# sglang-npu/DeepGEMM_Ascend

Hardware: AMD Instinct MI355X
Metric: fp8 TFLOPS + % MFMA peak, 4096^3 block-scaled GEMM; grouped-GEMM tok/s at 1/2/4/8 GPU (higher is better)
Workload: dtype bf16

## Files before the change

deepgemm_ascend_amd/csrc/dga_launch.hip:

```cpp
#include <hip/hip_runtime.h>
#include <atomic>
#include <cstdio>
#include <cstdlib>
#include <cstring>
#include <mutex>

#include "dga_hip.h"
#include "dga_internal.hpp"
#include "dga_fp8_menu_impl.hpp"
#include "gemm_fp8_aux_kernels.hpp"

namespace dga {

static std::atomic<int> g_last_hip_error{0};
int record_hip(hipError_t e)
{
    if (e != hipSuccess) {
        g_last_hip_error.store(static_cast<int>(e));
        return DGA_E_HIP;
    }
    return DGA_OK;
}
uint32_t device_cus()
{
    static std::atomic<uint32_t> cache[64];
    int dev = 0, n = 0;
    if (hipGetDevice(&dev) != hipSuccess || dev < 0 || dev >= 64) return 256;
    if (const uint32_t v = cache[dev].load()) return v;
    if (hipDeviceGetAttribute(&n, hipDeviceAttributeMultiprocessorCount, dev) != hipSuccess || n <= 0) return 256;
    cache[dev].store(static_cast<uint32_t>(n));
    return static_cast<uint32_t>(n);
}

struct Variant {
    int bm, bn, wm, wn;
    int (*launch)(const GemmParams &, hipStream_t);
    int lds;
    int (*launch_pp)(const GemmParams &, hipStream_t);
    int (*launch_cont)(const GemmParams &, hipStream_t);
    int stages = 2;
    int (*launch_lc)(const GemmParams &, hipStream_t) = nullptr;
    int (*launch_ps)(const GemmParams &, hipStream_t) = nullptr;
};

#define DGA_VARIANT(BM, BN, WM, WN) \
    Variant { BM, BN, WM, WN, &launch_cfg<GemmCfg<BM, BN, WM, WN>, 0>, GemmCfg<BM, BN, WM, WN>::LDS_BYTES, nullptr, nullptr }
#define DGA_VARIANT_C(BM, BN, WM, WN) \
    Variant { BM, BN, WM, WN, &launch_cfg<GemmCfg<BM, BN, WM, WN>, 0>, GemmCfg<BM, BN, WM, WN>::LDS_BYTES, nullptr, \
              &launch_cfg<GemmCfg<BM, BN, WM, WN>, 2> }
#define DGA_VARIANT_PP(BM, BN, WM, WN)                                                                       \
    Variant { BM, BN, WM, WN, &launch_cfg<GemmCfg<BM, BN, WM, WN>, 0>, GemmCfg<BM, BN, WM, WN>::LDS_BYTES, \
              &launch_cfg<GemmCfg<BM, BN, WM, WN>, 1>, &launch_cfg<GemmCfg<BM, BN, WM, WN>, 2> }

static const Variant kVariants[] = {
    DGA_VARIANT_PP(256, 256, 4, 2), DGA_VARIANT_C(128, 256, 2, 2), DGA_VARIANT_C(256, 128, 4, 1),
    DGA_VARIANT_C(128, 128, 2, 2), DGA_VARIANT_C(64, 256, 1, 4),  DGA_VARIANT(64, 128, 1, 4),
    DGA_VARIANT_C(128, 256, 2, 4),
    Variant{128, 256, 2, 4, &launch_cfg<GemmCfg<128, 256, 2, 4, 3>, 0>, GemmCfg<128, 256, 2, 4, 3>::LDS_BYTES, nullptr, nullptr, 3},
    Variant{128, 256, 2, 2, &launch_cfg<GemmCfg<128, 256, 2, 2, 3>, 0>, GemmCfg<128, 256, 2, 2, 3>::LDS_BYTES, nullptr, nullptr, 3,
            &launch_cfg<GemmCfg<128, 256, 2, 2, 3, 4>, 0>, &launch_persistent<GemmCfg<128, 256, 2, 2, 3, 4>>},
    Variant{128, 128, 2, 2, &launch_cfg<GemmCfg<128, 128, 2, 2, 3>, 0>, GemmCfg<128, 128, 2, 2, 3>::LDS_BYTES, nullptr, nullptr, 3,
            &launch_cfg<GemmCfg<128, 128, 2, 2, 3, 4>, 0>, &launch_persistent<GemmCfg<128, 128, 2, 2, 3, 4>>},
    Variant{64, 256, 1, 4, &launch_cfg<GemmCfg<64, 256, 1, 4, 3>, 0>, GemmCfg<64, 256, 1, 4, 3>::LDS_BYTES, nullptr, nullptr, 3,
            &launch_cfg<GemmCfg<64, 256, 1, 4, 3, 4>, 0>, &launch_persistent<GemmCfg<64, 256, 1, 4, 3, 4>>},

    DGA_VARIANT(32, 256, 1, 4),  DGA_VARIANT(32, 128, 1, 4),  DGA_VARIANT(16, 256, 1, 4),
    DGA_VARIANT(16, 128, 1, 4),
    Variant{64, 128, 1, 4, &launch_cfg<GemmCfg<64, 128, 1, 4, 3>, 0>, GemmCfg<64, 128, 1, 4, 3>::LDS_BYTES, nullptr, nullptr, 3,
            &launch_cfg<GemmCfg<64, 128, 1, 4, 3, 4>, 0>, &launch_persistent<GemmCfg<64, 128, 1, 4, 3, 4>>},
    Variant{32, 256, 1, 4, &launch_cfg<GemmCfg<32, 256, 1, 4, 3>, 0>, GemmCfg<32, 256, 1, 4, 3>::LDS_BYTES, nullptr, nullptr, 3},
    Variant{32, 128, 1, 4, &launch_cfg<GemmCfg<32, 128, 1, 4, 3>, 0>, GemmCfg<32, 128, 1, 4, 3>::LDS_BYTES, nullptr, nullptr, 3},
    Variant{16, 256, 1, 4, &launch_cfg<GemmCfg<16, 256, 1, 4, 3>, 0>, GemmCfg<16, 256, 1, 4, 3>::LDS_BYTES, nullptr, nullptr, 3},
    Variant{16, 128, 1, 4, &launch_cfg<GemmCfg<16, 128, 1, 4, 3>, 0>, GemmCfg<16, 128, 1, 4, 3>::LDS_BYTES, nullptr, nullptr, 3,
            &launch_cfg<GemmCfg<16, 128, 1, 4, 3, 4>, 0>, &launch_persistent<GemmCfg<16, 128, 1, 4, 3, 4>>},
};
static constexpr int kNumVariants = sizeof(kVariants) / sizeof(kVariants[0]);

struct Bf16xVariant {
    int bm, bn;
    int (*launch[3])(const GemmParams &, hipStream_t);
    int (*launch_kgroup)(const GemmParams &, hipStream_t);
};
#define DGA_BX_VARIANT(BM, BN, WM, WN) {BM, BN, {&launch_bf16x<GemmCfg<BM, BN, WM, WN, 3>>, &launch_bf16x_f32<GemmCfg<BM, BN, WM, WN, 3>>, \
                                         &launch_bf16x_rows<GemmCfg<BM, BN, WM, WN, 3>>}, &launch_bf16x_kgroup<GemmCfg<BM, BN, WM, WN, 3>>}
static const Bf16xVariant kBf16xVariants[] = {
    DGA_BX_VARIANT(128, 256, 2, 4), DGA_BX_VARIANT(128, 128, 2, 2), DGA_BX_VARIANT(64, 256, 1, 4), DGA_BX_VARIANT(64, 128, 1, 4),
    DGA_BX_VARIANT(32, 128, 1, 4),
};
static const Bf16xVariant *find_bf16x_variant(int m1, int n1)
{
    const int bm = m1 >= 128 ? 128 : (m1 >= 64 ? 64 : 32);
    const int bn = n1 >= 256 ? 256 : 128;
    for (const auto &v : kBf16xVariants)
        if (v.bm == bm && v.bn == bn) return &v;
    for (const auto &v : kBf16xVariants)
        if (v.bm == bm) return &v;
    return nullptr;
}

static const char *const kPolicyNames[] = {"fast", "bf16_exact", "strict", "fast_ue8m0", "bf16_exact_ue8m0", "auto"};
int default_policy()
{
    static const int v = [] {
        const char *e = std::getenv("DGA_DEFAULT_POLICY");
        if (!e || !*e) return 1;
        for (int i = 0; i < 6; ++i)
            if (!std::strcmp(e, kPolicyNames[i])) return i;
        return -1;
    }();
    return v;
}

int variant_count() { return kNumVariants; }
int variant_stages(int i) { return kVariants[i].stages; }
bool variant_has_loader_waves(int i) { return kVariants[i].launch_lc != nullptr; }
void variant_info(int i, int *bm, int *bn, int *wm, int *wn, int *lds)
{
    *bm = kVariants[i].bm; *bn = kVariants[i].bn; *wm = kVariants[i].wm; *wn = kVariants[i].wn;
    *lds = kVariants[i].lds;
}

static const Variant *find_variant(int bm, int bn, int wm, int wn, int stages)
{
    for (int i = 0; i < kNumVariants; ++i)
        if (kVariants[i].bm == bm && kVariants[i].bn == bn && (!wm || (kVariants[i].wm == wm && kVariants[i].wn == wn)) &&
            kVariants[i].stages == (stages == 3 ? 3 : 2))
            return &kVariants[i];
    if (stages == 3) return find_variant(bm, bn, wm, wn, 2);
    return wm ? find_variant(bm, bn, 0, 0, 2) : nullptr;
}

static int check_tiling(const dga_tiling_t &t)
{
    if (t.dispatchPolicyTag & ~(DGA_POLICY_UE8M0_SCALES | 7)) return DGA_E_TILING;
    const int tag = t.dispatchPolicyTag & 7;
    if (!known_kernel_serial(t.kernelSerial)) return DGA_E_TILING;
    if (t.k1 != 0 && t.k1 != 128) return DGA_E_TILING;
    if (t.splitkFactor > 1024) return DGA_E_RANGE;
    if (t.reserved0) return DGA_E_TILING;
    if (tag == DGA_POLICY_STRICT) return DGA_OK;
    if (t.m1 == 0 || t.n1 == 0) return DGA_E_TILING;
    if (!(t.stages == 0 || t.stages == 2 || t.stages == 3)) return DGA_E_TILING;
    const bool wsk = t.kernelSerial == DGA_KERNEL_SPLITK_WORKGROUP;
    if (t.build == DGA_BUILD_WSK_REGISTER && !wsk) return DGA_E_TILING;
    if (tag == DGA_POLICY_BF16_EXACT) {
        if (!find_bf16x_variant(t.m1, t.n1)) return DGA_E_TILING;
        switch (t.build) {
            case DGA_BUILD_DEFAULT: case DGA_BUILD_WSK_REGISTER: case DGA_BUILD_BX_AIMAGE: case DGA_BUILD_BX_IMAGE8: case DGA_BUILD_BX_IMAGE4:
            case DGA_BUILD_BX_PERSISTENT: case DGA_BUILD_BX_ONE_TILE: case DGA_BUILD_BX_GROUPED: break;
            case DGA_BUILD_BX_DECODE:
                if (!wsk || t.m1 != 64 || t.n1 != 128) return DGA_E_TILING;
                break;
            default: return DGA_E_TILING;
        }
        if ((t.kernelSerial == DGA_KERNEL_STREAMK_TAIL || t.kernelSerial == DGA_KERNEL_STREAMK_ONE_LAUNCH) && !(t.m1 >= 128 && t.n1 >= 256)) return DGA_E_TILING;
        return DGA_OK;
    }
    bool tile = false, grid = false;
    for (int i = 0; i < kNumVariants; ++i)
        if (kVariants[i].bm == t.m1 && kVariants[i].bn == t.n1) {
            tile = true;
            if (kVariants[i].wm == t.wavesM && kVariants[i].wn == t.wavesN) grid = true;
        }
    if (!tile) return DGA_E_TILING;
    if (t.m1 == 256 && t.n1 == 256 && t.wavesM == 2 && t.wavesN == 2 && (t.dispatchPolicyTag & DGA_POLICY_UE8M0_SCALES) &&
        (tag == DGA_POLICY_CONTINUOUS || tag == DGA_POLICY_CONTINUOUS_PERSISTENT))
        grid = true;
    if ((t.wavesM || t.wavesN) && !grid) return DGA_E_TILING;
    if (t.build != DGA_BUILD_DEFAULT && t.build != DGA_BUILD_WSK_REGISTER) return DGA_E_TILING;
    if (tag == DGA_POLICY_PINGPONG && !(t.m1 == 256 && t.n1 == 256)) return DGA_E_TILING;
    if ((t.kernelSerial == DGA_KERNEL_STREAMK_TAIL || t.kernelSerial == DGA_KERNEL_STREAMK_ONE_LAUNCH) && !(t.m1 == 256 && t.n1 == 256))
        return DGA_E_TILING;
    return DGA_OK;
}

static int (*find_clock_build(const Variant *v, int policy))(const GemmParams &, hipStream_t)
{
    if (v->bm == 256 && v->bn == 256 && policy == DGA_POLICY_CONTINUOUS) return &launch_cfg<GemmCfg<256, 256, 4, 2, 2>, 2, true>;
    if (v->bm == 128 && v->bn == 256 && v->stages == 3 && policy == DGA_POLICY_LOADER_WAVES) return &launch_cfg<GemmCfg<128, 256, 2, 2, 3, 4>, 0, true>;
    return nullptr;
}

struct Switches {
    int bf16_exact = env_int("DGA_BF16_EXACT", 0);
    int strict = env_int("DGA_STRICT", 0);
    int b_nt = env_int("DGA_B_NT", -1), out_nt = env_int("DGA_OUT_NT", -1);
    int unaligned = env_int("DGA_UNALIGNED", -1);
    int xcd_remap = env_int("DGA_XCD_REMAP", 1);
    int bx_image = env_int("DGA_BX_IMAGE", -1);
    int wsk = env_int("DGA_WSK", -1), wsk_dma = env_int("DGA_WSK_DMA", -1);
    int pingpong = env_int("DGA_PINGPONG", -1);
    int bx_persist = env_int("DGA_BF16X_PERSIST", -1), bx_grouped = env_int("DGA_BX_GROUPED", -1);
};
static const Switches &env()
{
    static const Switches s;
    return s;
}

static int strict_bm(int groups, int m, int n)
{
    const int64_t tiles64 = static_cast<int64_t>(groups) * ((m + 63) / 64) * ((n + 127) / 128);
    return (m > 32 && tiles64 >= static_cast<int64_t>(device_cus())) ? 64 : 32;
}

static bool partial_overlap(const float *c, const float *out, uintptr_t bytes)
{
    if (!c || c == out) return false;
    const uintptr_t co = reinterpret_cast<uintptr_t>(c), oo = reinterpret_cast<uintptr_t>(out);
    return co < oo + bytes && oo < co + bytes;
}

static dga_problem_t fp8_problem(int m, int n, int k, int groups)
{
    dga_problem_t pr{};
    pr.m = m; pr.n = n; pr.k = k; pr.groups = groups;
    pr.layoutTagA = DGA_LAYOUT_ROW_MAJOR; pr.layoutTagB = DGA_LAYOUT_COLUMN_MAJOR;
    pr.layoutTagC = DGA_LAYOUT_ROW_MAJOR; pr.dtype = DGA_DT_FP8_E4M3FN;
    return pr;
}

static int check_tiling_for(Out kind, const dga_tiling_t *t)
{
    if (kind == Out::F32Rows) return dga_tiling_check_wgrad(t);
    if (kind == Out::F32) return dga_tiling_check_fp32_out(t);
    return check_tiling(*t);
}

struct Carver {
    uint8_t *ws;
    size_t bytes, used = 0;
    uint8_t *operator()(size_t n)
    {
        const size_t at = (used + 255) & ~size_t(255);
        if (!ws || at + n > bytes) return nullptr;
        used = at + n;
        return ws + at;
    }
};


static int resolve_tiling(const Fp8Call &c, dga_tiling_t &local)
{
    dga_problem_t pr = fp8_problem(c.m, c.n, c.k, c.groups);
    pr.expected_m = c.expected_m;
    pr.flags = c.m_indices ? DGA_PROBLEM_CONTIGUOUS_M : 0;
    if (c.kind == Out::F32) return dga_tiling_fp32_out(&pr, &local);
    if (c.kind == Out::F32Rows) return dga_tiling_wgrad(&pr, &local);
    const int default_policy = dga::default_policy();
    if (default_policy < 0) return DGA_E_RANGE;
    const int rc = (env().bf16_exact || default_policy == 1 || default_policy == 4) ? dga_tiling_bf16_exact(&pr, &local) : dga_tiling(&pr, &local);
    if (rc != DGA_OK) return rc;
    if (default_policy == 5 && c.groups == 1 && !c.m_indices) {
        dga_tiling_t tb;
        if (dga_tiling_bf16_exact(&pr, &tb) == DGA_OK && tb.kernelSerial == DGA_KERNEL_SPLITK_WORKGROUP) local = tb;
    }
    if (default_policy == 2) local.dispatchPolicyTag = DGA_POLICY_STRICT;
    if (default_policy == 3 || default_policy == 4) local.dispatchPolicyTag |= DGA_POLICY_UE8M0_SCALES;
    return DGA_OK;
}

static int fill_params(const Fp8Call &c, GemmParams &p)
{
    const int m = c.m, n = c.n, k = c.k;
    p.a = static_cast<const uint8_t *>(c.a);
    p.sfa = c.sfa;
    p.b = static_cast<const uint8_t *>(c.b);
    p.sfb = c.sfb;
    p.out = static_cast<uint16_t *>(c.out);
    p.masked_m = c.masked_m;
    p.m_indices = c.m_indices;
    p.b_groups = c.b_groups;
    p.m = m; p.n = n; p.k = k;
    p.kb_n = (k + 127) / 128;
    p.nb_n = c.kind == Out::F32Rows ? n : (n + 127) / 128;
    p.lda = k; p.ldb = k; p.ldc = n;
    p.a_gs = static_cast<int64_t>(m) * k;
    p.b_gs = static_cast<int64_t>(n) * k;
    p.c_gs = static_cast<int64_t>(m) * n;
    p.sfa_gs = static_cast<int64_t>(m) * p.kb_n;
    p.sfb_gs = static_cast<int64_t>(p.nb_n) * p.kb_n;
    p.sfa_ld = p.kb_n;
    if (const Fp8Strided *sd = c.sd) {
        if (c.groups != 1 || c.b_groups != 1 || c.masked_m || c.m_indices || c.ix || c.clock_stamps) return DGA_E_SHAPE;
        if (sd->lda < k || sd->ldb < k) return DGA_E_SHAPE;
        if ((sd->lda != k && (sd->lda & 15)) || (sd->ldb != k && (sd->ldb & 15))) return DGA_E_ALIGN;
        p.lda = sd->lda; p.ldb = sd->ldb;
    }
    if (const Fp8Indexed *ix = c.ix) {
        if (!ix->row_index || ix->lda < k || ix->ldc < n || ix->sfa_ld < p.kb_n || ix->rows < 0) return DGA_E_SHAPE;
        p.row_index = ix->row_index;
        p.lda = ix->lda; p.ldc = ix->ldc; p.sfa_ld = ix->sfa_ld;
        p.a_gs = p.c_gs = p.sfa_gs = 0;
        p.a_bytes = ix->rows * ix->lda;
        if (p.a_bytes >= 0x7FFFFFFFll) return DGA_E_RANGE;
    }
    p.groups = c.groups;
    const bool weight_stream = c.groups > 1 ? (c.masked_m && !c.m_indices)
                                            : (c.m_indices && c.b_groups > 1 && static_cast<int64_t>(m) <= static_cast<int64_t>(c.b_groups) * DGA_CONTIGUOUS_M_ALIGNMENT);
    p.b_nt = env().b_nt >= 0 ? env().b_nt : (weight_stream ? 1 : 0);
    p.out_nt = env().out_nt >= 0 ? env().out_nt : (weight_stream ? 1 : 0);
    p.splitk = 1;
    p.stamps = c.clock_stamps;
    if (c.kind != Out::Bf16) p.c_in = c.c_in;
    return DGA_OK;
}

static int run_strict(const Fp8Call &c, GemmParams &p)
{
    int bm = strict_bm(c.groups, c.m, c.n);
    if (static_cast<int64_t>(c.groups) * ((c.m + bm - 1) / bm) * ((c.n + 127) / 128) > 0x7FFFFFFFll) return DGA_E_SHAPE;
    const int64_t tiles128 = static_cast<int64_t>((c.m + 127) / 128) * ((c.n + 127) / 128);
    if (c.groups == 1 && !c.masked_m && !c.m_indices && !c.ix && tiles128 >= 2 * static_cast<int64_t>(device_cus())) bm = 128;
    p.tiles_m = (c.m + bm - 1) / bm;
    p.tiles_n = (c.n + 127) / 128;
    const unsigned grid = static_cast<unsigned>(static_cast<int64_t>(c.groups) * p.tiles_m * p.tiles_n);
    hipLaunchKernelGGL(strict_kernel(bm, c.kind), dim3(grid), dim3(256), 0, c.stream, p);
    return record_hip(hipGetLastError());
}

static int try_unaligned(const Fp8Call &c, const dga_tiling_t &t, const GemmParams &p)
{
    const int m = c.m, n = c.n, k = c.k;
    if (k > 0 && (k % 16) != 0 && !c.ix && !c.sd && c.groups == 1 && !c.masked_m && !c.m_indices && !c.clock_stamps && !env().bf16_exact &&
        t.dispatchPolicyTag != DGA_POLICY_BF16_EXACT &&
        (env().unaligned >= 0 ? env().unaligned != 0
                              : (t.kernelSerial == DGA_KERNEL_PADDING_COMMON ||
                                 !c.workspace || c.workspace_bytes < (((static_cast<size_t>(m) * p.kb_n * 128 + 255) & ~size_t(255)) +
                                                                      static_cast<size_t>(n) * p.kb_n * 128 + 256)))) {
        GemmParams q = p;
        q.tiles_m = (m + 127) / 128;
        q.tiles_n = (n + 255) / 256;
        q.raster_group = t.swizzleOffset ? t.swizzleOffset : 1;
        q.xcd_remap = env().xcd_remap;
        return launch_unaligned(q, c.stream);
    }
    return DGA_E_TILING;
}

static int pad_operands(const Fp8Call &c, GemmParams &p, Carver &carve, int &k)
{
    const int m = c.m, n = c.n;
    if (c.sd && k > 0) {
        const int k16 = (k + 15) & ~15;
        auto in_place = [&](const void *base, int64_t ld, int flag) {
            return (reinterpret_cast<uintptr_t>(base) & 15) == 0 && (ld & 15) == 0 && ld >= k16 && ((k % 16) == 0 || (c.sd->flags & flag));
        };
        const bool a_ok = in_place(p.a, p.lda, DGA_ROWS_A_ZERO_PADDED), b_ok = in_place(p.b, p.ldb, DGA_ROWS_B_ZERO_PADDED);
        bool ready = a_ok && b_ok;
        if (!ready) {
            const int kp = p.kb_n * 128;
            uint8_t *pa = a_ok ? nullptr : carve(static_cast<size_t>(m) * kp);
            uint8_t *pb = b_ok ? nullptr : carve(static_cast<size_t>(n) * kp);
            if ((a_ok || pa) && (b_ok || pb)) {
                const int st = pad_rows_strided(a_ok ? nullptr : p.a, p.lda, pa, a_ok ? 0 : m, b_ok ? nullptr : p.b, p.ldb, pb,
                                                b_ok ? 0 : n, k, kp, c.stream);
                if (st != DGA_OK) return st;
                if (!a_ok) { p.a = pa; p.lda = kp; }
                if (!b_ok) { p.b = pb; p.ldb = kp; }
                ready = true;
            }
        }
        if (ready) { p.k = k16; k = k16; }
    } else
    if (k > 0 && (k % 16) != 0 && !c.ix) {
        const int kp = p.kb_n * 128;
        const int64_t rows_a = static_cast<int64_t>(c.groups) * m, rows_b = static_cast<int64_t>(c.b_groups) * n;
        uint8_t *pa = carve(static_cast<size_t>(rows_a) * kp);
        uint8_t *pb = pa ? carve(static_cast<size_t>(rows_b) * kp) : nullptr;
        if (pa && pb && ((reinterpret_cast<uintptr_t>(pa) | reinterpret_cast<uintptr_t>(pb)) & 15) == 0) {
            const int st = pad_rows(p.a, pa, rows_a, p.b, pb, rows_b, k, kp, c.stream);
            if (st != DGA_OK) return st;
            p.a = pa; p.b = pb;
            p.k = kp; p.lda = kp; p.ldb = kp;
            p.a_gs = static_cast<int64_t>(m) * kp;
            p.b_gs = static_cast<int64_t>(n) * kp;
            k = kp;
        }
    }
    return DGA_OK;
}

static bool split_k(const Fp8Call &c, const dga_tiling_t &t, const Variant *v, const Bf16xVariant *vx, int bx_image, bool bx_ue8m0,
                    const GemmParams &p, Carver &carve, int &rc)
{
    if (t.splitkFactor <= 1 || c.groups != 1 || c.masked_m || c.m_indices) return false;
    int s = t.splitkFactor;
    const int kbps = (p.kb_n + s - 1) / s;
    s = (p.kb_n + kbps - 1) / kbps;
    float *slabs = s > 1 ? reinterpret_cast<float *>(carve(static_cast<size_t>(s) * c.m * c.n * sizeof(float))) : nullptr;
    if (!slabs) return false;
    GemmParams pk = p;
    pk.splitk = s;
    pk.kb_per_split = kbps;
    pk.partial = slabs;
    pk.groups = s;
    const int64_t mn = static_cast<int64_t>(c.m) * c.n;
    const dim3 grid(static_cast<unsigned>((mn / 8 + 255) / 256 + 1));
    if (c.kind != Out::Bf16) {
        rc = vx->launch[static_cast<int>(c.kind == Out::F32Rows ? Out::F32Rows : Out::Bf16)](pk, c.stream);
        if (rc != DGA_OK) return true;
        hipLaunchKernelGGL(splitk_reduce_f32_kernel, grid, dim3(256), 0, c.stream, slabs, p.c_in, static_cast<float *>(c.out), mn, s);
        rc = record_hip(hipGetLastError());
        return true;
    }
    rc = DGA_E_TILING;
    if (vx && bx_ue8m0 && !bx_image) rc = launch_bf16u(vx->bm, vx->bn, pk, c.stream);
    if (rc == DGA_E_TILING)
        rc = vx ? (bx_image ? launch_bf16x_image(pk, bx_image, c.stream) : vx->launch[0](pk, c.stream)) : v->launch(pk, c.stream);
    if (rc != DGA_OK) return true;
    hipLaunchKernelGGL(splitk_reduce_bf16_kernel, grid, dim3(256), 0, c.stream, slabs, p.out, mn, s);
    rc = record_hip(hipGetLastError());
    return true;
}

static int run_bf16x(const Fp8Call &c, const dga_tiling_t &t, const Bf16xVariant *vx, int bx_image, bool bx_ue8m0, GemmParams &p,
                     Carver &carve)
{
    const bool dense = c.groups == 1 && !c.masked_m && !c.m_indices && !c.ix;
    const int form = static_cast<int>(c.kind);
    if (!bx_ue8m0 && dense && c.kind != Out::F32Rows && t.kernelSerial == DGA_KERNEL_SPLITK_WORKGROUP && t.build == DGA_BUILD_BX_DECODE) {
        const int64_t dsk_tiles = static_cast<int64_t>((c.m + 63) / 64) * ((c.n + 127) / 128);
        const int s = bx_dsk_splits(dsk_tiles, p.kb_n, t.splitkFactor, static_cast<int>(device_cus()));
        const size_t need = s > 0 ? bx_dsk_workspace_bytes(dsk_tiles, s) : 0;
        uint8_t *dsk_ws = need ? carve(need) : nullptr;
        if (s > 0 && (need == 0 || dsk_ws)) {
            const int rc = launch_bf16x_dsk(p, s, dsk_ws, need, c.stream, c.kind);
            if (rc != DGA_E_TILING) return rc;
        }
    }
    if (dense && c.kind != Out::F32Rows && t.build != DGA_BUILD_BX_DECODE &&
        (env().wsk >= 0 ? env().wsk != 0 : t.kernelSerial == DGA_KERNEL_SPLITK_WORKGROUP)) {
        const int rc = launch_wsk_dma(p, c.stream, 1, c.kind);
        if (rc != DGA_E_TILING) return rc;
    }
    int rc;
    if (split_k(c, t, nullptr, vx, bx_image, bx_ue8m0, p, carve, rc)) return rc;
    if (bx_ue8m0 && !bx_image && t.kernelSerial != DGA_KERNEL_STREAMK_TAIL) {
        rc = launch_bf16u(vx->bm, vx->bn, p, c.stream);
        if (rc != DGA_E_TILING) return rc;
    }
    if (bx_image) return launch_bf16x_image(p, bx_image, c.stream);
    if (t.kernelSerial == DGA_KERNEL_STREAMK_TAIL && dense && vx->bm == 128 && vx->bn == 256) {
        const PartialRound pr = partial_round(p.tiles_m * p.tiles_n, device_cus(), 2);
        const Bf16xVariant *vq = find_bf16x_variant(64, 128);
        if (pr && vq && vq->bm == 64 && vq->bn == 128) {
            GemmParams pm = p;
            pm.launch_tiles = static_cast<int>(pr.main_tiles);
            rc = launch_bf16x_persistent(pm, c.kind, c.stream);
            if (rc == DGA_E_TILING) rc = vx->launch[form](pm, c.stream);
            if (rc != DGA_OK) return rc;
            GemmParams pt = p;
            pt.tail_begin = static_cast<int>(pr.main_tiles);
            pt.tail_sub = 2;
            pt.launch_tiles = static_cast<int>(pr.tail * 4);
            return vq->launch[form](pt, c.stream);
        }
    }
    const int64_t tiles = static_cast<int64_t>(p.groups) * p.tiles_m * p.tiles_n, cus = static_cast<int64_t>(device_cus());
    if (t.kernelSerial == DGA_KERNEL_STREAMK_ONE_LAUNCH && vx->bm == 128 && vx->bn == 256 && dense && c.kind != Out::F32Rows) {
        const size_t need = bx_streamk_workspace_bytes(device_cus());
        if (uint8_t *sk_ws = carve(need)) {
            rc = launch_bf16x_streamk(p, sk_ws, need, c.stream, c.kind);
            if (rc != DGA_E_TILING) return rc;
        }
    }
    if (vx->bm == 128 && vx->bn == 256 && !c.m_indices && c.kind == Out::Bf16 &&
        (env().bx_grouped >= 0 ? (env().bx_grouped != 0 && c.masked_m) : t.build == DGA_BUILD_BX_GROUPED)) {
        rc = launch_bf16x_grouped(p, c.stream);
        if (rc != DGA_E_TILING) return rc;
    }
    const bool pays = tiles > cus;
    if (vx->bm == 128 && vx->bn == 256 &&
        (env().bx_persist >= 0 ? env().bx_persist != 0 : (t.build == DGA_BUILD_BX_PERSISTENT || (t.build != DGA_BUILD_BX_ONE_TILE && pays)))) {
        rc = launch_bf16x_persistent(p, c.kind, c.stream);
        if (rc != DGA_E_TILING) return rc;
    }
    return vx->launch[form](p, c.stream);
}

static int run_fast(const Fp8Call &c, const dga_tiling_t &t, const Variant *v, bool ue8m0, GemmParams &p, Carver &carve)
{
    const bool dense = c.groups == 1 && !c.masked_m && !c.m_indices && !c.ix;
    const hipStream_t stream = c.stream;
    if (!c.clock_stamps && dense && (env().wsk >= 0 ? env().wsk != 0 : t.kernelSerial == DGA_KERNEL_SPLITK_WORKGROUP)) {
        if (env().wsk_dma >= 0 ? env().wsk_dma != 0 : t.build != DGA_BUILD_WSK_REGISTER) {
            const int rc = launch_wsk_dma(p, stream);
            if (rc != DGA_E_TILING) return rc;
        }
        const int rc = launch_wsk(p, stream);
        if (rc != DGA_E_TILING) return rc;
    }
    if (c.clock_stamps && (t.splitkFactor > 1 || t.kernelSerial == DGA_KERNEL_STREAMK_TAIL)) return DGA_E_TILING;
    int rc;
    if (split_k(c, t, v, nullptr, 0, false, p, carve, rc)) return rc;
    const int policy = env().pingpong >= 0 ? env().pingpong : t.dispatchPolicyTag;
    auto launch_main = [&](const GemmParams &q) -> int {
        const bool runs_persistent = policy == DGA_POLICY_PERSISTENT && v->launch_ps && q.splitk <= 1 && !q.tail_sub && q.launch_tiles == 0;
        if (ue8m0 && !q.stamps && !runs_persistent) {
            const bool cont = (policy == DGA_POLICY_CONTINUOUS || policy == DGA_POLICY_CONTINUOUS_PERSISTENT) && v->launch_cont;
            const bool loaders = (policy == DGA_POLICY_LOADER_WAVES || policy == DGA_POLICY_PERSISTENT) && v->launch_lc;
            if (cont && v->bm == 256 && v->bn == 256 && t.wavesM == 2 && t.wavesN == 2 && !q.tail_sub) {
                const int r4 = launch_ue8m0_w4(q, stream);
                if (r4 != DGA_E_TILING) return r4;
            }
            const int rc = launch_ue8m0(v->bm, v->bn, loaders, cont, q, stream);
            if (rc != DGA_E_TILING) return rc;
        }
        if (q.stamps) {
            auto clk = find_clock_build(v, (policy == 2 || policy == DGA_POLICY_CONTINUOUS_PERSISTENT) && v->launch_cont ? 2 : (policy == DGA_POLICY_LOADER_WAVES && v->launch_lc ? policy : 0));
            return clk ? clk(q, stream) : DGA_E_TILING;
        }
        if (policy == DGA_POLICY_PERSISTENT && v->launch_ps && q.splitk <= 1 && !q.tail_sub && q.launch_tiles == 0)
            return v->launch_ps(q, stream);
        if ((policy == DGA_POLICY_LOADER_WAVES || policy == DGA_POLICY_PERSISTENT) && v->launch_lc) return v->launch_lc(q, stream);
        if (policy == 1 && v->launch_pp) return v->launch_pp(q, stream);
        if (policy == DGA_POLICY_CONTINUOUS_PERSISTENT && v->bm == 256 && v->bn == 256 && v->launch_cont) {
            const int rc = launch_cont_persistent(q, stream);
            return rc == DGA_E_TILING ? v->launch_cont(q, stream) : rc;
        }
        if ((policy == 2 || policy == DGA_POLICY_CONTINUOUS_PERSISTENT) && v->launch_cont) return v->launch_cont(q, stream);
        return v->launch(q, stream);
    };

    if (t.kernelSerial == DGA_KERNEL_STREAMK_ONE_LAUNCH && !c.clock_stamps && dense && v->bm == 256 && v->bn == 256) {
        const size_t need = streamk_workspace_bytes(device_cus());
        if (uint8_t *sk_ws = carve(need)) {
            rc = launch_streamk(p, sk_ws, need, ue8m0, stream);
            if (rc != DGA_E_TILING) return rc;
        }
    }

    if (t.kernelSerial == DGA_KERNEL_STREAMK_TAIL && c.groups == 1 && !c.masked_m && !c.m_indices && v->bm == 256 && v->bn == 256) {
        const PartialRound pr = partial_round(p.tiles_m * p.tiles_n, device_cus(), 2);
        const Variant *vq = find_variant(128, 128, 0, 0, 3);
        if (pr && vq) {
            GemmParams pm = p;
            pm.launch_tiles = static_cast<int>(pr.main_tiles);
            rc = launch_main(pm);
            if (rc != DGA_OK) return rc;
            GemmParams pt = p;
            pt.tail_begin = static_cast<int>(pr.main_tiles);
            pt.tail_sub = 2;
            pt.launch_tiles = static_cast<int>(pr.tail * 4);
            if (ue8m0) {
                const int rq = launch_ue8m0(128, 128, vq->launch_lc != nullptr, false, pt, stream);
                if (rq != DGA_E_TILING) return rq;
            }
            if (vq->launch_lc) return vq->launch_lc(pt, stream);
            return vq->launch(pt, stream);
        }
    }
    return launch_main(p);
}

int run_fp8(const Fp8Call &c)
{
    if (c.kind != Out::Bf16 && (c.groups != 1 || c.b_groups != 1 || c.masked_m || c.m_indices || c.ix || c.clock_stamps)) return DGA_E_SHAPE;
    if (c.m < 0 || c.n < 0 || c.k < 0 || c.groups < 0 || c.b_groups < 0) return DGA_E_SHAPE;
    if (c.groups == 0 || c.m == 0 || c.n == 0) return DGA_OK;
    if (!c.a || !c.b || !c.sfa || !c.sfb || !c.out) {
        if (!c.out || c.k != 0) return DGA_E_NULL;
    }
    dga_tiling_t local;
    const dga_tiling_t *tiling = c.tiling;
    if (!tiling) {
        if (int rc = resolve_tiling(c, local)) return rc;
        tiling = &local;
    }
    if (int rc = check_tiling_for(c.kind, tiling)) return rc;
    dga_tiling_t unflagged;
    bool ue8m0 = false, bx_ue8m0 = false;
    if (tiling->dispatchPolicyTag & DGA_POLICY_UE8M0_SCALES) {
        unflagged = *tiling;
        unflagged.dispatchPolicyTag &= static_cast<uint8_t>(~DGA_POLICY_UE8M0_SCALES);
        ue8m0 = unflagged.dispatchPolicyTag != DGA_POLICY_STRICT && unflagged.dispatchPolicyTag != DGA_POLICY_BF16_EXACT &&
                unflagged.dispatchPolicyTag != DGA_POLICY_PINGPONG;
        bx_ue8m0 = unflagged.dispatchPolicyTag == DGA_POLICY_BF16_EXACT;
        tiling = &unflagged;
    }
    if (c.workspace && dga_workspace_bytes(tiling) > c.workspace_bytes) return DGA_E_WORKSPACE;
    if (c.m_indices && tiling->m1 != 2 * DGA_CONTIGUOUS_M_ALIGNMENT &&
        (tiling->m1 == 0 || tiling->m1 > DGA_CONTIGUOUS_M_ALIGNMENT || DGA_CONTIGUOUS_M_ALIGNMENT % tiling->m1))
        return DGA_E_TILING;
    GemmParams p{};
    if (int rc = fill_params(c, p)) return rc;

    const bool strict = tiling->dispatchPolicyTag == DGA_POLICY_STRICT || env().strict;
    if (c.clock_stamps && (strict || (c.k % 16) != 0)) return DGA_E_TILING;
    if (strict) return run_strict(c, p);
    if (int rc = try_unaligned(c, *tiling, p); rc != DGA_E_TILING) return rc;
    Carver carve{static_cast<uint8_t *>(c.workspace), c.workspace_bytes};
    int k = c.k;
    if (int rc = pad_operands(c, p, carve, k)) return rc;

    const bool fast_ok = (k % 16 == 0) && k > 0 && ((reinterpret_cast<uintptr_t>(p.a) & 15) == 0) &&
                         ((reinterpret_cast<uintptr_t>(p.b) & 15) == 0) && (p.lda % 16 == 0) && (p.ldb % 16 == 0) &&
                         (static_cast<int64_t>(p.lda) * 257 < 0x7FFFFFFFll) && (static_cast<int64_t>(p.ldb) * 257 < 0x7FFFFFFFll);
    if (!fast_ok) {
        const auto generic = c.kind == Out::F32Rows ? gemm_fp8_blockscaled_nt_generic_kernel<1, 1>
                             : c.kind == Out::F32   ? gemm_fp8_blockscaled_nt_generic_kernel<1>
                                                    : gemm_fp8_blockscaled_nt_generic_kernel<>;
        hipLaunchKernelGGL(generic, dim3((c.n + 15) / 16, (c.m + 15) / 16, c.groups), dim3(256), 0, c.stream, p);
        return record_hip(hipGetLastError());
    }
    const bool bf16x = tiling->dispatchPolicyTag == DGA_POLICY_BF16_EXACT || env().bf16_exact;
    const Bf16xVariant *vx = bf16x ? find_bf16x_variant(tiling->m1, tiling->n1) : nullptr;
    if (bf16x && (!vx || c.clock_stamps)) return DGA_E_TILING;
    int bx_image = 0;
    if (vx && vx->bm == 128 && vx->bn == 256 && !c.m_indices && !c.ix && c.kind == Out::Bf16) {
        const int e = env().bx_image;
        if (e >= 0) bx_image = e == 4 ? 4 : (e == 1 ? 1 : (e ? 8 : 0));
        else if (tiling->build == DGA_BUILD_BX_AIMAGE) bx_image = 1;
        else if (tiling->build == DGA_BUILD_BX_IMAGE8) bx_image = 8;
        else if (tiling->build == DGA_BUILD_BX_IMAGE4) bx_image = 4;
    }
    const Variant *v = find_variant(tiling->m1, tiling->n1, tiling->wavesM, tiling->wavesN, tiling->stages);
    if (!v && !vx) return DGA_E_TILING;
    const int tile_m = vx ? vx->bm : v->bm, tile_n = vx ? vx->bn : v->bn;
    const bool wants_loaders = tiling->dispatchPolicyTag == DGA_POLICY_LOADER_WAVES || tiling->dispatchPolicyTag == DGA_POLICY_PERSISTENT;
    if (!vx && wants_loaders && !v->launch_lc)
        for (int i = 0; i < kNumVariants; ++i)
            if (kVariants[i].bm == v->bm && kVariants[i].bn == v->bn && kVariants[i].stages == v->stages && kVariants[i].launch_lc) {
                v = &kVariants[i];
                break;
            }
    p.tiles_m = (c.m + tile_m - 1) / tile_m;
    p.tiles_n = (c.n + tile_n - 1) / tile_n;
    if (env().out_nt < 0 && c.groups == 1 && !c.masked_m && !c.m_indices && !c.ix && c.kind == Out::Bf16 &&
        static_cast<int64_t>(p.tiles_m) * p.tiles_n <= 2 * static_cast<int64_t>(device_cus()))
        p.out_nt = 2;
    p.raster_group = tiling->swizzleOffset ? tiling->swizzleOffset : 1;
    p.xcd_remap = env().xcd_remap;
    return vx ? run_bf16x(c, *tiling, vx, bx_image, bx_ue8m0, p, carve) : run_fast(c, *tiling, v, ue8m0, p, carve);
}

}

extern "C" {

int dga_default_policy(char *name_out, int cap)
{
    const int v = dga::default_policy();
    if (v < 0) return DGA_E_RANGE;
    if (name_out && cap > 0) {
        std::strncpy(name_out, dga::kPolicyNames[v], static_cast<size_t>(cap) - 1);
        name_out[cap - 1] = 0;
    }
    return DGA_OK;
}

int dga_tiling_check(const dga_tiling_t *tiling)
{
    if (!tiling) return DGA_E_NULL;
    return dga::check_tiling(*tiling);
}

int dga_tiling_check_fp32_out(const dga_tiling_t *tiling)
{
    if (!tiling) return DGA_E_NULL;
    if (int rc = dga::check_tiling(*tiling)) return rc;
    const int tag = tiling->dispatchPolicyTag;
    if (tag != DGA_POLICY_BF16_EXACT && tag != DGA_POLICY_STRICT) return DGA_E_TILING;
    if (tag == DGA_POLICY_STRICT) return DGA_OK;
    switch (tiling->build) {
        case DGA_BUILD_BX_AIMAGE: case DGA_BUILD_BX_IMAGE8: case DGA_BUILD_BX_IMAGE4: case DGA_BUILD_BX_GROUPED: return DGA_E_TILING;
        default: return DGA_OK;
    }
}

int dga_tiling_check_wgrad(const dga_tiling_t *tiling)
{
    if (int rc = dga_tiling_check_fp32_out(tiling)) return rc;
    if (tiling->dispatchPolicyTag == DGA_POLICY_STRICT) return DGA_OK;
    if (tiling->kernelSerial == DGA_KERNEL_SPLITK_WORKGROUP || tiling->kernelSerial == DGA_KERNEL_STREAMK_ONE_LAUNCH ||
        tiling->build == DGA_BUILD_BX_DECODE || tiling->build == DGA_BUILD_WSK_REGISTER)
        return DGA_E_TILING;
    return DGA_OK;
}

static int fp32_out_entry(const void *a, int64_t lda, const float *sfa, const void *b, int64_t ldb, const float *sfb, const float *c,
                          float *out, int m, int n, int k, int flags, const dga_tiling_t *tiling, void *workspace,
                          size_t workspace_bytes, void *stream, dga::Out kind)
{
    if (m < 0 || n < 0 || k < 0) return DGA_E_SHAPE;
    if (m == 0 || n == 0) return DGA_OK;
    if (!out) return DGA_E_NULL;
    if (dga::partial_overlap(c, out, static_cast<uintptr_t>(m) * static_cast<uintptr_t>(n) * sizeof(float))) return DGA_E_SHAPE;
    if (tiling)
        if (int rc = dga::check_tiling_for(kind, tiling)) return rc;
    const dga::Fp8Strided sd{lda, ldb, flags};
    dga::Fp8Call call{a, sfa, b, sfb, out, m, n, k, tiling, workspace, workspace_bytes, static_cast<hipStream_t>(stream)};
    if (lda != k || ldb != k) call.sd = &sd;
    call.kind = kind;
    call.c_in = c;
    return dga::run_fp8(call);
}

int dga_gemm_fp8_fp8_fp32_nt(const void *a, int64_t lda, const float *sfa, const void *b, int64_t ldb, const float *sfb, const float *c,
                             float *out, int m, int n, int k, int flags, const dga_tiling_t *tiling, void *workspace,
                             size_t workspace_bytes, void *stream)
{
    return fp32_out_entry(a, lda, sfa, b, ldb, sfb, c, out, m, n, k, flags, tiling, workspace, workspace_bytes, stream, dga::Out::F32);
}

int dga_wgrad_gemm_fp8_fp8_fp32_nt(const void *a, int64_t lda, const float *sfa, const void *b, int64_t ldb, const float *sfb,
                                   const float *c, float *out, int m, int n, int k, int flags, const dga_tiling_t *tiling,
                                   void *workspace, size_t workspace_bytes, void *stream)
{
    return fp32_out_entry(a, lda, sfa, b, ldb, sfb, c, out, m, n, k, flags, tiling, workspace, workspace_bytes, stream, dga::Out::F32Rows);
}

int dga_tiling_check_k_grouped_wgrad(const dga_tiling_t *tiling)
{
    if (int rc = dga_tiling_check_wgrad(tiling)) return rc;
    if (tiling->splitkFactor > 1) return DGA_E_TILING;
    if (tiling->dispatchPolicyTag == DGA_POLICY_STRICT) return DGA_OK;
    if (tiling->kernelSerial != DGA_KERNEL_COMMON && tiling->kernelSerial != DGA_KERNEL_SMALL && tiling->kernelSerial != DGA_KERNEL_PADDING_COMMON)
        return DGA_E_TILING;
    if (tiling->build != DGA_BUILD_DEFAULT && tiling->build != DGA_BUILD_BX_PERSISTENT && tiling->build != DGA_BUILD_BX_ONE_TILE)
        return DGA_E_TILING;
    const dga::Bf16xVariant *vx = dga::find_bf16x_variant(tiling->m1, tiling->n1);
    if (!vx || vx->bm != tiling->m1 || vx->bn != tiling->n1) return DGA_E_TILING;
    if (tiling->build == DGA_BUILD_BX_PERSISTENT && !(tiling->m1 == 128 && tiling->n1 == 256)) return DGA_E_TILING;
    return DGA_OK;
}

int dga_k_grouped_wgrad_gemm_fp8_fp8_fp32_nt(const void *a, int64_t lda, const float *sfa, const void *b, int64_t ldb, const float *sfb,
                                             const float *c, float *out, const int32_t *ks, int groups, int m, int n, int k_total,
                                             int flags, const dga_tiling_t *tiling, void *workspace, size_t workspace_bytes,
                                             void *stream)
{
    (void)workspace; (void)workspace_bytes;
    if (m < 0 || n < 0 || k_total < 0 || groups < 0 || k_total % 128) return DGA_E_SHAPE;
    if (flags & ~(DGA_ROWS_A_ZERO_PADDED | DGA_ROWS_B_ZERO_PADDED)) return DGA_E_SHAPE;
    if (groups == 0 || m == 0 || n == 0) return DGA_OK;
    if (k_total > 0) {
        if (lda < k_total || ldb < k_total) return DGA_E_SHAPE;
        if ((lda & 15) || (ldb & 15)) return DGA_E_ALIGN;
        if (static_cast<int64_t>(m) * lda >= 0x7FFFFFFFll || static_cast<int64_t>(n) * ldb >= 0x7FFFFFFFll) return DGA_E_RANGE;
    }
    if (!out || !ks || (k_total > 0 && (!a || !b || !sfa || !sfb))) return DGA_E_NULL;
    const int64_t elems = static_cast<int64_t>(groups) * m * n;
    if (dga::partial_overlap(c, out, static_cast<uintptr_t>(elems) * sizeof(float))) return DGA_E_SHAPE;
    dga_tiling_t local;
    if (!tiling) {
        dga_problem_t pr = dga::fp8_problem(m, n, k_total, groups);
        if (int rc = dga_tiling_k_grouped_wgrad(&pr, &local)) return rc;
        tiling = &local;
    }
    if (int rc = dga_tiling_check_k_grouped_wgrad(tiling)) return rc;
    dga::GemmParams p{};
    p.a = static_cast<const uint8_t *>(a); p.sfa = sfa;
    p.b = static_cast<const uint8_t *>(b); p.sfb = sfb;
    p.out = reinterpret_cast<uint16_t *>(out);
    p.c_in = c;
    p.ks = ks;
    p.m = m; p.n = n; p.k = k_total;
    p.kb_n = k_total / 128;
    p.nb_n = n;
    p.lda = k_total ? lda : 0; p.ldb = k_total ? ldb : 0; p.ldc = n;
    p.c_gs = static_cast<int64_t>(m) * n;
    p.sfa_ld = p.kb_n;
    p.groups = groups;
    p.splitk = 1;
    p.raster_group = tiling->swizzleOffset ? tiling->swizzleOffset : 1;
    p.xcd_remap = 1;
    const hipStream_t st = static_cast<hipStream_t>(stream);
    if (tiling->dispatchPolicyTag == DGA_POLICY_STRICT) {
        const int bm = dga::strict_bm(groups, m, n);
        p.tiles_m = (m + bm - 1) / bm;
        p.tiles_n = (n + 127) / 128;
        if (static_cast<int64_t>(groups) * p.tiles_m * p.tiles_n > 0x7FFFFFFFll) return DGA_E_SHAPE;
        return dga::launch_strict_kgroup(p, bm, st);
    }
    const dga::Bf16xVariant *vx = dga::find_bf16x_variant(tiling->m1, tiling->n1);
    if (!vx) return DGA_E_TILING;
    p.tiles_m = (m + vx->bm - 1) / vx->bm;
    p.tiles_n = (n + vx->bn - 1) / vx->bn;
    const int64_t tiles = static_cast<int64_t>(groups) * p.tiles_m * p.tiles_n;
    if (tiles > 0x7FFFFFFFll) return DGA_E_SHAPE;
    if (vx->bm == 128 && vx->bn == 256 &&
        (tiling->build == DGA_BUILD_BX_PERSISTENT || (tiling->build == DGA_BUILD_DEFAULT && tiles > static_cast<int64_t>(dga::device_cus()))))
        return dga::launch_bf16x_persistent_kgroup(p, st);
    return vx->launch_kgroup(p, st);
}

int dga_gemm_fp8_fp8_bf16_nt(const void *a, const float *sfa, const void *b, const float *sfb, void *out, int m,
                             int n, int k, const dga_tiling_t *tiling, void *workspace, size_t workspace_bytes,
                             void *stream)
{
    return dga::run_fp8({a, sfa, b, sfb, out, m, n, k, tiling, workspace, workspace_bytes, static_cast<hipStream_t>(stream)});
}

int dga_gemm_fp8_fp8_bf16_nt_strided(const void *a, int64_t lda, const float *sfa, const void *b, int64_t ldb, const float *sfb,
                                     void *out, int m, int n, int k, int flags, const dga_tiling_t *tiling, void *workspace,
                                     size_t workspace_bytes, void *stream)
{
    const dga::Fp8Strided sd{lda, ldb, flags};
    dga::Fp8Call call{a, sfa, b, sfb, out, m, n, k, tiling, workspace, workspace_bytes, static_cast<hipStream_t>(stream)};
    call.sd = &sd;
    return dga::run_fp8(call);
}

int dga_m_grouped_gemm_fp8_fp8_bf16_nt_masked(const void *a, const float *sfa, const void *b, const float *sfb,
                                              void *out, const int32_t *masked_m, int groups, int m_max, int n,
                                              int k, int expected_m, const dga_tiling_t *tiling, void *workspace,
                                              size_t workspace_bytes, void *stream)
{
    if (groups > 0 && m_max > 0 && !masked_m) return DGA_E_NULL;
    dga::Fp8Call call{a, sfa, b, sfb, out, m_max, n, k, tiling, workspace, workspace_bytes, static_cast<hipStream_t>(stream)};
    call.groups = call.b_groups = groups;
    call.expected_m = expected_m;
    call.masked_m = masked_m;
    return dga::run_fp8(call);
}

int dga_m_grouped_gemm_fp8_fp8_bf16_nt_contiguous(const void *a, const float *sfa, const void *b, const float *sfb,
                                                  void *out, const int32_t *m_indices, int m_sum, int groups, int n,
                                                  int k, const dga_tiling_t *tiling, void *workspace,
                                                  size_t workspace_bytes, void *stream)
{
    if (groups < 0) return DGA_E_SHAPE;
    if (m_sum > 0 && n > 0 && groups > 0 && !m_indices) return DGA_E_NULL;
    if (groups == 0) return DGA_OK;
    dga::Fp8Call call{a, sfa, b, sfb, out, m_sum, n, k, tiling, workspace, workspace_bytes, static_cast<hipStream_t>(stream)};
    call.b_groups = groups;
    call.m_indices = m_indices;
    return dga::run_fp8(call);
}

int dga_m_grouped_gemm_fp8_fp8_bf16_nt_masked_indexed(const void *a, int64_t lda, const float *sfa, int64_t sfa_ld,
                                                      const void *b, const float *sfb, void *out, int64_t ldc,
                                                      const int64_t *row_index, int64_t rows, const int32_t *masked_m,
                                                      int groups, int m_max, int n, int k, int expected_m,
                                                      const dga_tiling_t *tiling, void *workspace, size_t workspace_bytes,
                                                      void *stream)
{
    if (groups > 0 && m_max > 0 && (!masked_m || !row_index)) return DGA_E_NULL;
    const dga::Fp8Indexed ix{row_index, lda, sfa_ld, ldc, rows};
    dga::Fp8Call call{a, sfa, b, sfb, out, m_max, n, k, tiling, workspace, workspace_bytes, static_cast<hipStream_t>(stream)};
    call.groups = call.b_groups = groups;
    call.expected_m = expected_m;
    call.masked_m = masked_m;
    call.ix = &ix;
    return dga::run_fp8(call);
}

int dga_last_hip_error(void) { return dga::g_last_hip_error.load(); }

int dga_device_platform(dga_platform_t *out)
{
    if (!out) return DGA_E_NULL;
    dga_platform_mi355x(out);
    int dev = 0;
    hipDeviceProp_t prop;
    if (hipGetDevice(&dev) != hipSuccess || hipGetDeviceProperties(&prop, dev) != hipSuccess) return DGA_E_HIP;
    out->coreNum = static_cast<uint32_t>(prop.multiProcessorCount);
    out->l1Size = prop.maxSharedMemoryPerMultiProcessor ? prop.maxSharedMemoryPerMultiProcessor : out->l1Size;
    out->waveSize = static_cast<uint32_t>(prop.warpSize);
    return DGA_OK;
}

}
```

deepgemm_ascend_amd/csrc/dga_launch_menu_l.hip:

```cpp
#include <cstdlib>
#include "dga_fp8_menu_impl.hpp"
#include "gemm_fp8_bf16x_grouped_kernel.hpp"
namespace dga {

template <bool KTAIL, bool BNT, bool STAG, bool IDX = false>
static int launch_bf16x_grouped_one(const GemmParams &p, hipStream_t stream)
{
    typedef GemmCfg<128, 256, 2, 4, 3> Cfg;
    constexpr int kLds = Cfg::LDS_BYTES + (IDX ? 256 * 16 : 0);
    const int64_t tiles = static_cast<int64_t>(p.groups) * p.tiles_m * p.tiles_n;
    const unsigned grid = static_cast<unsigned>(std::min<int64_t>(tiles, device_cus()));
    return launch_kernel<gemm_fp8_bf16x_grouped_kernel<KTAIL, BNT, STAG, IDX>>(grid, Cfg::NT, kLds, stream, p);
}

int launch_bf16x_grouped(const GemmParams &p, hipStream_t stream)
{
    if (p.tail_sub || p.m_indices || p.launch_tiles > 0 || p.splitk > 1 || p.kb_n < 2) return DGA_E_TILING;
    const bool nt = p.b_nt != 0;
#ifdef DGA_BXG_KNOBS
    if (const char *e = std::getenv("DGA_BXG_KNOB"); e && (std::atoi(e) & 2)) {
        if (p.k % 128) return nt ? launch_bf16x_grouped_one<true, true, false>(p, stream) : launch_bf16x_grouped_one<true, false, false>(p, stream);
        return nt ? launch_bf16x_grouped_one<false, true, false>(p, stream) : launch_bf16x_grouped_one<false, false, false>(p, stream);
    }
#endif
    if (p.row_index) {
        if (p.k % 128) return nt ? launch_bf16x_grouped_one<true, true, true, true>(p, stream) : launch_bf16x_grouped_one<true, false, true, true>(p, stream);
        return nt ? launch_bf16x_grouped_one<false, true, true, true>(p, stream) : launch_bf16x_grouped_one<false, false, true, true>(p, stream);
    }
    if (p.k % 128) return nt ? launch_bf16x_grouped_one<true, true, true>(p, stream) : launch_bf16x_grouped_one<true, false, true>(p, stream);
    return nt ? launch_bf16x_grouped_one<false, true, true>(p, stream) : launch_bf16x_grouped_one<false, false, true>(p, stream);
}
}
```

deepgemm_ascend_amd/csrc/gemm_fp8_bf16x_grouped_kernel.hpp:

```cpp
#pragma once
#include "gemm_fp8_kernel.hpp"

namespace dga {

template <bool KTAIL, bool BNT, bool STAGGER = true, bool INDEXED = false>
__global__ void __launch_bounds__(512) __attribute__((amdgpu_waves_per_eu(2, 2)))
gemm_fp8_bf16x_grouped_kernel(const GemmParams p)
{
    typedef GemmCfg<128, 256, 2, 4, 3> Cfg;
    constexpr int BM = Cfg::kBM, BN = Cfg::kBN, WN = Cfg::kWN, TM = Cfg::TM, TN = Cfg::TN, DNT = Cfg::DNT;
    constexpr int NL = Cfg::LOADS_PER_STAGE, LAGT = 2, RING = 4, NT = Cfg::NT;
    static_assert(Cfg::NT == 512 && DNT == 512 && TM == 4 && TN == 4 && Cfg::SC_ITERS == 1 && Cfg::STAGES == 3, "the grouped schedule");
    typedef __bf16 v8bf __attribute__((ext_vector_type(8)));
    extern __shared__ __attribute__((aligned(16))) uint8_t smem[];

    const int tid = threadIdx.x, lane = tid & 63;
    const int wave = __builtin_amdgcn_readfirstlane(tid >> 6);
    const int wm = wave / WN, wn = wave % WN;
    const int li = lane & 15, kg = lane >> 4;
    const int KB = p.kb_n;

    const int tiles_per_group = p.tiles_m * p.tiles_n;
    const int total = p.groups * tiles_per_group;
    int first = 0, count = total, step = gridDim.x, slot = blockIdx.x;
    if (p.xcd_remap) {
        const int xcd = blockIdx.x & 7, q = total >> 3, r = total & 7;
        first = xcd < r ? xcd * (q + 1) : r * (q + 1) + (xcd - r) * q;
        count = q + (xcd < r ? 1 : 0);
        step = ((int)gridDim.x - xcd + 7) >> 3;
        slot = blockIdx.x >> 3;
    }
    struct Tile { int g, M, m0, n0; };
    typedef const __attribute__((address_space(4))) int32_t *const_i32_ptr;
    const const_i32_ptr masked_m_c = (const_i32_ptr)p.masked_m;
    auto seek = [&](int &local, Tile &t) -> bool {
        for (; local < count; local += step) {
            const int tile = first + local;
            const int g = tile / tiles_per_group;
            const int t_in = tile - g * tiles_per_group;
            const int gm = p.raster_group;
            const int per = gm * p.tiles_n;
            const int band = t_in / per;
            const int row0 = band * gm;
            const int rows = min(p.tiles_m - row0, gm);
            const int loc = t_in - band * per;
            const int tm = row0 + loc % rows, tn = loc / rows;
            const int M = p.masked_m ? min(masked_m_c[g], p.m) : p.m;
            const int m0 = tm * BM;
            if (m0 >= M) continue;
            t.g = g; t.M = M; t.m0 = m0; t.n0 = tn * BN;
            return true;
        }
        return false;
    };

    const uint32_t lds0 = (uint32_t)(uintptr_t)(lptr_t)smem;
    constexpr uint32_t kOutOfRange = 0x80000000u;
    const int a_col = ((tid & 7) ^ swz_a(tid >> 3)) * 16;
    const int b_col = ((tid & 7) ^ swz_b(tid >> 3)) * 16;
    v4i a_rsrc, b_rsrc;
    uint32_t a_voff[Cfg::A_ITERS], b_voff[Cfg::B_ITERS];
    const float *sc_src;
    int kbf = 0;
    bool fill_valid = true;
    constexpr bool indexed = INDEXED;
    static_assert(Cfg::A_ITERS == 2, "partner slot: two A offsets and the scale pointer");
    uint32_t *const pslot = reinterpret_cast<uint32_t *>(smem + Cfg::LDS_BYTES) + (tid & (DNT / 2 - 1)) * 4;
    auto a_off_of = [&](const Tile &t, int it, int td) -> uint32_t {
        const int row = (it * DNT + td) >> 3;
        if (row >= t.M - t.m0) return kOutOfRange;
        const uint32_t r = indexed ? (uint32_t)p.row_index[(int64_t)t.g * p.m + t.m0 + row] : (uint32_t)row;
        return r * (uint32_t)p.lda + a_col;
    };
    auto b_off_of = [&](const Tile &t, int it, int td) -> uint32_t {
        const int row = (it * DNT + td) >> 3;
        return (uint32_t)min(row, p.n - 1 - t.n0) * (uint32_t)p.ldb + b_col;
    };
    auto sc_of = [&](const Tile &t, int td) -> const float * {
        const float *SFA = p.sfa + (int64_t)t.g * p.sfa_gs, *SFB = p.sfb + (int64_t)t.g * p.sfb_gs;
        if (td >= BM) return SFB + (int64_t)min(t.n0 / 128 + min(td - BM, 7), p.nb_n - 1) * p.kb_n;
        const int mr = min(t.m0 + td, t.M - 1);
        return SFA + (indexed ? p.row_index[(int64_t)t.g * p.m + mr] : (int64_t)mr) * p.sfa_ld;
    };
    Tile T{}, F{};
    auto set_fill = [&](const Tile &t) {
        a_rsrc = indexed ? make_rsrc(p.a, p.a_bytes)
                         : make_rsrc(p.a + (int64_t)t.g * p.a_gs + (int64_t)t.m0 * p.lda, (int64_t)(t.M - t.m0) * p.lda);
        b_rsrc = make_rsrc(p.b + (int64_t)t.g * p.b_gs + (int64_t)t.n0 * p.ldb, (int64_t)(p.n - t.n0) * p.ldb);
#pragma unroll
        for (int it = 0; it < Cfg::A_ITERS; ++it) a_voff[it] = a_off_of(t, it, tid);
#pragma unroll
        for (int it = 0; it < Cfg::B_ITERS; ++it) b_voff[it] = b_off_of(t, it, tid);
        sc_src = sc_of(t, tid);
        if constexpr (INDEXED) {
            if (wm == 1) {
                const uint64_t ps = (uint64_t)(uintptr_t)sc_of(t, tid - DNT / 2);
                *reinterpret_cast<v4i *>(pslot) = v4i{(int)a_off_of(t, 0, tid - DNT / 2), (int)a_off_of(t, 1, tid - DNT / 2), (int)(uint32_t)ps, (int)(uint32_t)(ps >> 32)};
            }
        }
    };
    auto refill = [&](int idx, int stage, auto sc) {
        constexpr int S = decltype(sc)::value;
        const int w = wave - 4 * S, td = tid - S * (DNT / 2);
        const uint32_t sa = lds0 + stage * Cfg::STAGE_BYTES + w * 1024;
        const int k0 = kbf * 128;
        if (idx < Cfg::A_ITERS) {
            uint32_t voff = fill_valid ? (S ? (INDEXED ? pslot[idx] : a_off_of(F, idx, td)) : a_voff[idx]) : kOutOfRange;
            if constexpr (KTAIL) voff = (k0 + a_col < p.k) ? voff : kOutOfRange;
            dma16(voff, a_rsrc, (uint32_t)k0, sa + idx * DNT * 16);
        } else if (idx < Cfg::A_ITERS + Cfg::B_ITERS) {
            const int it = idx - Cfg::A_ITERS;
            uint32_t voff = fill_valid ? (S ? b_off_of(F, it, td) : b_voff[it]) : kOutOfRange;
            if constexpr (KTAIL) voff = (k0 + b_col < p.k) ? voff : kOutOfRange;
            if constexpr (BNT) dma16_nt(voff, b_rsrc, (uint32_t)k0, sa + Cfg::A_BYTES + it * DNT * 16);
            else dma16(voff, b_rsrc, (uint32_t)k0, sa + Cfg::A_BYTES + it * DNT * 16);
        } else {
            const float *src = S ? (INDEXED ? reinterpret_cast<const float *>((uintptr_t)*reinterpret_cast<const uint64_t *>(pslot + 2)) : sc_of(F, td)) : sc_src;
            dma4(src + (fill_valid ? kbf : KB - 1), lds0 + stage * Cfg::STAGE_BYTES + Cfg::A_BYTES + Cfg::B_BYTES + w * 256);
        }
    };
    constexpr std::integral_constant<int, 0> kOwn{};
    constexpr std::integral_constant<int, 1> kPartner{};

    const int a_row = wm * (BM / Cfg::kWM) + li;
    const int a_off0 = a_row * 128 + ((kg ^ swz_a(a_row)) * 16);
    const int a_off1 = a_row * 128 + (((kg + 4) ^ swz_a(a_row)) * 16);
    const int b_row = wn * (BN / WN) + 8 * (li >> 2) + (li & 3);
    const int b_off0 = Cfg::A_BYTES + b_row * 128 + ((kg ^ swz_b(b_row)) * 16);
    const int b_off1 = Cfg::A_BYTES + b_row * 128 + (((kg + 4) ^ swz_b(b_row)) * 16);
    const int sa_off = Cfg::A_BYTES + Cfg::B_BYTES + (wm * (BM / Cfg::kWM) + li) * 4;
    const int sb_off = Cfg::A_BYTES + Cfg::B_BYTES + (BM + (wn * (BN / WN)) / 128) * 4;

    v4f acc[TM][TN];
    v4f part[RING];
    v4i afx[TM][4], bfx[2][4];
    v4i braw[2], araw[2][2];
    float s_cur[TM], s_old[TM];

    auto wait_all_but = [&](auto base, int extra) {
        constexpr int B = decltype(base)::value;
        if (extra >= 8) wait_vmcnt<B + 8>();
        else if (extra >= 6) wait_vmcnt<B + 6>();
        else if (extra >= 4) wait_vmcnt<B + 4>();
        else if (extra >= 2) wait_vmcnt<B + 2>();
        else wait_vmcnt<B>();
    };
    auto wait_landed = [&](int younger, int extra) {
        if (younger >= 2 * NL) wait_all_but(std::integral_constant<int, 2 * NL>{}, extra);
        else if (younger >= NL) wait_all_but(std::integral_constant<int, NL>{}, extra);
        else wait_all_but(std::integral_constant<int, 0>{}, extra);
    };

    int local = slot;
    if (!seek(local, T)) return;
    F = T;
    set_fill(F);
#pragma unroll
    for (int d = 0; d < 2; ++d) {
#pragma unroll
        for (int idx = 0; idx < NL; ++idx) refill(idx, d, kOwn);
        ++kbf;
    }
    int cur = 0;
    DGA_STAMP_DECL
    DGA_STAMP_CLOCK(6, 7);
    DGA_STAMP_START();
    int stores_pending = 0;
    int younger = NL;

    auto advance_fill = [&]() {
        if (kbf == KB) {
            local += step;
            fill_valid = seek(local, F);
            if (fill_valid) set_fill(F);
            kbf = 0;
        }
    };

    auto run_tile = [&](auto Lc, auto lonec, auto stagc) __attribute__((always_inline)) {
        constexpr int L = decltype(Lc)::value;
        constexpr bool lone = decltype(lonec)::value;
        constexpr bool STAG = decltype(stagc)::value;
        constexpr int G = 4 * (L > 0 ? L : 1);
        constexpr int TILES = (L > 0 ? L : 1) * TN;
        constexpr int SP = L > 0 ? L : 1;
        constexpr int HALF = 2 * TILES;
        static_assert(1 + (NL - 1) * SP < HALF, "the refill fits half a block");
        static_assert(!(STAG && (lone || L == 0)), "a staggered wave multiplies and issues its own pieces");
        if constexpr (L > 0) {
#pragma unroll
            for (int i = 0; i < L; ++i)
#pragma unroll
                for (int j = 0; j < TN; ++j) acc[i][j] = v4f{0.f, 0.f, 0.f, 0.f};
#pragma unroll
            for (int i = 0; i < RING; ++i) part[i] = v4f{0.f, 0.f, 0.f, 0.f};
#pragma unroll
            for (int i = 0; i < L; ++i) s_old[i] = 0.f;
        }
        auto head = [&](const uint8_t *sc) __attribute__((always_inline)) {
            araw[0][0] = *(const v4i *)(sc + a_off0);
            araw[0][1] = *(const v4i *)(sc + a_off1);
            braw[0] = *(const v4i *)(sc + b_off0);
            braw[1] = *(const v4i *)(sc + b_off1);
            if constexpr (L > 1) {
                araw[1][0] = *(const v4i *)(sc + a_off0 + 2048);
                araw[1][1] = *(const v4i *)(sc + a_off1 + 2048);
            }
            const float sfb0 = *(const float *)(sc + sb_off);
            float sa[L > 0 ? L : 1];
#pragma unroll
            for (int i = 0; i < L; ++i) sa[i] = *(const float *)(sc + sa_off + i * 64);
            __builtin_amdgcn_sched_barrier(0);
#pragma unroll
            for (int c = 0; c < 8; ++c) bx_convert(braw, bfx[0], c);
            braw[0] = *(const v4i *)(sc + b_off0 + b_frag_off(1));
#pragma unroll
            for (int c = 8; c < 16; ++c) bx_convert(braw, bfx[0], c);
            braw[1] = *(const v4i *)(sc + b_off1 + b_frag_off(1));
#pragma unroll
            for (int c = 0; c < 16; ++c) bx_convert(araw[0], afx[0], c);
            if constexpr (L > 2) {
                araw[0][0] = *(const v4i *)(sc + a_off0 + 2 * 2048);
                araw[0][1] = *(const v4i *)(sc + a_off1 + 2 * 2048);
            }
#pragma unroll
            for (int i = 0; i < L; ++i) s_cur[i] = sa[i] * sfb0;
            __builtin_amdgcn_sched_barrier(0);
        };
        auto gaps = [&](auto u0c, auto u1c, auto refillc, const uint8_t *sc, int fill) __attribute__((always_inline)) {
            constexpr int U0 = decltype(u0c)::value, U1 = decltype(u1c)::value;
            constexpr bool REFILL = decltype(refillc)::value;
#pragma unroll
            for (int u = U0; u < U1; ++u) {
                const int t = u >> 2, q = u & 3, nt = t / L, mt = t % L, g = u % G;
                part[t % RING] = __builtin_amdgcn_mfma_f32_16x16x32_bf16(
                    __builtin_bit_cast(v8bf, bfx[nt & 1][q]), __builtin_bit_cast(v8bf, afx[mt][q]),
                    q == 0 ? v4f{0.f, 0.f, 0.f, 0.f} : part[t % RING], 0, 0, 0);
                __builtin_amdgcn_sched_barrier(0);
                if (REFILL && u - U0 >= 1 && (u - U0 - 1) % SP == 0 && (u - U0 - 1) / SP < NL) refill((u - U0 - 1) / SP, fill, kOwn);
                if (nt == 0 && mt + 1 < L) {
#pragma unroll
                    for (int c = 0; c < 4; ++c) bx_convert(araw[(mt + 1) & 1], afx[mt + 1], 4 * q + c);
                    if (q == 3 && mt + 3 < L) {
                        araw[(mt + 1) & 1][0] = *(const v4i *)(sc + a_off0 + (mt + 3) * 2048);
                        araw[(mt + 1) & 1][1] = *(const v4i *)(sc + a_off1 + (mt + 3) * 2048);
                    }
                }
                if (nt + 1 < TN) {
#pragma unroll
                    for (int c = 16 * g / G; c < 16 * (g + 1) / G; ++c) bx_convert(braw, bfx[(nt + 1) & 1], c);
                    if (nt + 2 < TN) {
                        if (g == G / 2 - 1) braw[0] = *(const v4i *)(sc + b_off0 + b_frag_off(nt + 2));
                        if (g == G - 1) braw[1] = *(const v4i *)(sc + b_off1 + b_frag_off(nt + 2));
                    }
                }
                {
                    const int j = t >= LAGT ? t - LAGT : TILES + t - LAGT, jn = j / L, jm = j % L;
                    const float sv = t >= LAGT ? s_cur[jm] : s_old[jm];
                    acc[jm][jn][q] = __builtin_fmaf(part[j % RING][q], sv, acc[jm][jn][q]);
                }
                __builtin_amdgcn_sched_barrier(0);
            }
        };
        constexpr std::integral_constant<int, 0> kU0{};
        constexpr std::integral_constant<int, HALF> kUh{};
        constexpr std::integral_constant<int, 4 * TILES> kU1{};
        auto end_of_block = [&]() {
#pragma unroll
            for (int i = 0; i < L; ++i) s_old[i] = s_cur[i];
        };
        auto top = [&](int kb) __attribute__((always_inline)) -> int {
            DGA_STAMP(0);
            wait_landed(younger, kb < 2 ? stores_pending : 0);
            DGA_STAMP(1);
            __builtin_amdgcn_s_barrier();
            asm volatile("" ::: "memory");
            DGA_STAMP(2);
            advance_fill();
            return cur >= 1 ? cur - 1 : 2;
        };
        auto next_block = [&]() {
            ++kbf;
            cur = cur == 2 ? 0 : cur + 1;
        };
        if constexpr (STAG) {
            {
                const int fill = top(0);
                younger = NL;
#pragma unroll
                for (int idx = 0; idx < NL; ++idx) refill(idx, fill, kOwn);
                const uint8_t *sc = smem + cur * Cfg::STAGE_BYTES;
                head(sc);
                gaps(kU0, kUh, std::false_type{}, sc, fill);
                next_block();
            }
            for (int kb = 1; kb < KB; ++kb) {
                const int fill = top(kb);
                const uint8_t *sc = smem + cur * Cfg::STAGE_BYTES;
                gaps(kUh, kU1, std::true_type{}, sc, fill);
                end_of_block();
                head(sc);
                DGA_STAMP(3);
                gaps(kU0, kUh, std::false_type{}, sc, fill);
                DGA_STAMP(4);
                next_block();
            }
            gaps(kUh, kU1, std::false_type{}, smem, 0);
            end_of_block();
        } else {
            for (int kb = 0; kb < KB; ++kb) {
                const int fill = top(kb);
                if constexpr (L == 0) {
#pragma unroll
                    for (int idx = 0; idx < NL; ++idx) {
                        if (lone) refill(idx, fill, kPartner);
                        refill(idx, fill, kOwn);
                    }
                    younger = lone ? 2 * NL : NL;
                } else {
                    younger = lone ? 0 : NL;
                    const uint8_t *sc = smem + cur * Cfg::STAGE_BYTES;
                    head(sc);
                    DGA_STAMP(3);
                    if constexpr (lone) gaps(kU0, kU1, std::false_type{}, sc, fill);
                    else gaps(kU0, kU1, std::true_type{}, sc, fill);
                    end_of_block();
                    DGA_STAMP(4);
                }
                next_block();
            }
        }
        stores_pending = 0;
        if constexpr (L > 0) {
#pragma unroll
            for (int t = 0; t < LAGT; ++t) {
                const int j = TILES + t - LAGT, jn = j / L, jm = j % L;
#pragma unroll
                for (int q = 0; q < 4; ++q) acc[jm][jn][q] = __builtin_fmaf(part[j % RING][q], s_old[jm], acc[jm][jn][q]);
            }
            uint16_t *C = p.out + (int64_t)T.g * p.c_gs;
            const int m_row = T.m0 + wm * (BM / Cfg::kWM) + li;
            const int n_base = T.n0 + wn * (BN / WN) + 8 * kg;
            const bool vec_ok = ((p.ldc & 7) == 0) && ((((uintptr_t)C) & 15) == 0);
            if (vec_ok && T.n0 + BN <= p.n) stores_pending = 2 * L;
#pragma unroll
            for (int mt = 0; mt < L; ++mt) {
                const int m = m_row + mt * 16;
                if (m >= T.M) continue;
                uint16_t *crow = C + (indexed ? p.row_index[(int64_t)T.g * p.m + m] : (int64_t)m) * p.ldc;
#pragma unroll
                for (int j = 0; j < TN / 2; ++j) {
                    const int n = n_base + 32 * j;
                    const v4f lo = acc[mt][2 * j], hi = acc[mt][2 * j + 1];
                    const v2bf h0 = __builtin_convertvector(v2f{lo.x, lo.y}, v2bf);
                    const v2bf h1 = __builtin_convertvector(v2f{lo.z, lo.w}, v2bf);
                    const v2bf h2 = __builtin_convertvector(v2f{hi.x, hi.y}, v2bf);
                    const v2bf h3 = __builtin_convertvector(v2f{hi.z, hi.w}, v2bf);
                    const v4i pk = v4i{__builtin_bit_cast(int, h0), __builtin_bit_cast(int, h1),
                                       __builtin_bit_cast(int, h2), __builtin_bit_cast(int, h3)};
                    if (vec_ok && n + 8 <= p.n) {
                        if (p.out_nt == 1) asm volatile("global_store_dwordx4 %0, %1, off nt" :: "v"(crow + n), "v"(pk) : "memory");
                        else if (p.out_nt == 2) asm volatile("global_store_dwordx4 %0, %1, off sc0 sc1" :: "v"(crow + n), "v"(pk) : "memory");
                        else if (p.out_nt == 3) asm volatile("global_store_dwordx4 %0, %1, off sc0 sc1 nt" :: "v"(crow + n), "v"(pk) : "memory");
                        else asm volatile("global_store_dwordx4 %0, %1, off" :: "v"(crow + n), "v"(pk) : "memory");
                    } else {
                        const uint16_t *e = (const uint16_t *)&pk;
#pragma unroll
                        for (int q = 0; q < 8; ++q)
                            if (n + q < p.n) crow[n + q] = e[q];
                    }
                }
            }
        }
    };

    for (;;) {
        const int rows = T.M - T.m0 - wm * (BM / Cfg::kWM);
        const int L = rows <= 0 ? 0 : (rows >= 64 ? 4 : (rows + 15) >> 4);
        const bool lone = T.M - T.m0 <= BM / Cfg::kWM;
        constexpr std::true_type yes{};
        constexpr std::false_type no{};
        if (lone) {
            if (L == 0) run_tile(std::integral_constant<int, 0>{}, yes, no);
            else if (L == 1) run_tile(std::integral_constant<int, 1>{}, yes, no);
            else if (L == 2) run_tile(std::integral_constant<int, 2>{}, yes, no);
            else if (L == 3) run_tile(std::integral_constant<int, 3>{}, yes, no);
            else run_tile(std::integral_constant<int, 4>{}, yes, no);
        } else if (wm == 0) {
            run_tile(std::integral_constant<int, 4>{}, no, no);
        } else {
            constexpr std::integral_constant<bool, STAGGER> st{};
            if (L == 1) run_tile(std::integral_constant<int, 1>{}, no, st);
            else if (L == 2) run_tile(std::integral_constant<int, 2>{}, no, st);
            else if (L == 3) run_tile(std::integral_constant<int, 3>{}, no, st);
            else run_tile(std::integral_constant<int, 4>{}, no, st);
        }
        if (!fill_valid) break;
        T = F;
    }
    DGA_STAMP(5);
    DGA_STAMP_CLOCK(6, 7);
    DGA_STAMP_FLUSH();
    wait_vmcnt<0>();
}

}
```

deepgemm_ascend_amd/harness/sweep.py:

```python
from __future__ import annotations

import argparse
import json
import os
from dataclasses import asdict, dataclass, field
from pathlib import Path

import torch

SHAPE_GROUP = [
    [4096, 4096, 4096], [8, 7168, 18432], [8, 18432, 7168], [64, 4096, 7168], [64, 7168, 18432], [64, 18432, 7168],
    [64, 24576, 1536], [64, 32768, 512], [64, 7168, 16384], [128, 4096, 7168], [128, 7168, 18432], [128, 18432, 7168],
    [1024, 4096, 7168], [1024, 18432, 7168], [2048, 4096, 7168], [1279, 5003, 7681], [3511, 6151, 8191], [5119, 6997, 9901],
]
TILES = [(256, 256), (128, 256), (256, 128), (128, 128), (64, 256), (64, 128), (32, 256), (32, 128), (16, 256), (16, 128)]
RASTERS = [1, 2, 4, 8, 16]
ERROR_TOL = 1e-4


@dataclass
class Result:
    idx: int
    M: int
    N: int
    K: int
    time: float
    diff: float
    negative: bool
    parameters: dict = field(default_factory=dict)


THREE_STAGE = {(128, 256), (128, 128), (64, 256), (64, 128), (32, 256), (32, 128), (16, 256), (16, 128)}
LOADER_WAVES = {(128, 256), (128, 128), (64, 256), (64, 128), (16, 128)}
PINGPONG = {(256, 256)}


def heuristic_raster(m, n, bm, bn, splitk=1, xcds=8, stages=2):
    tiles_m = -(-m // bm)
    lds = (max(bm, 32) * 128 + bn * 128 + ((bm + 8 + 255) // 256) * 256 * 4) * (3 if stages == 3 else 2)
    waves = 8 if (bm, bn) == (256, 256) else 4
    wg_per_cu = max(1, min(160 * 1024 // lds, 2048 // (waves * 64)))
    conc = min(max(1, (tiles_m * -(-n // bn) * splitk) // xcds), 32 * wg_per_cu)
    gm = 1
    while (gm * 2) * (gm * 2) <= conc and gm * 2 <= tiles_m:
        gm *= 2
    return min(gm, 255)


def grid_shapes(count, seed=0, max_mnk=2 ** 39):
    import random
    rng = random.Random(seed)
    out = []
    while len(out) < count:
        m = int(round(2 ** rng.uniform(3, 13)))
        if rng.random() < 0.5:
            m = max(8, (m + 15) // 16 * 16)
        n = max(512, int(round(2 ** rng.uniform(9, 14))) // 128 * 128)
        k = max(512, int(round(2 ** rng.uniform(9, 14))) // 128 * 128)
        if m * n * k <= max_mnk and [m, n, k] not in out:
            out.append([m, n, k])
    return out


def candidates(m, n, k, rasters=None):
    out = []
    kb = -(-k // 128)
    for bm, bn in TILES:
        if bm >= 2 * max(m, 16) and bm > 16:
            continue
        blocks = -(-m // bm) * -(-n // bn)
        splits = [1] + [s for s in (2, 3, 4, 5, 6, 8, 16) if blocks * s <= 1024 and kb // s >= 4 and blocks < 192]
        for r in (RASTERS if rasters is None else [0]):
            if r > max(1, -(-m // bm)):
                continue
            for st in ([2, 3] if (bm, bn) in THREE_STAGE else [2]):
                for sk in splits:
                    lw = ([0, 4, 5] if sk == 1 and blocks > CUS else [0, 4]) if st == 3 and (bm, bn) in LOADER_WAVES else [0]
                    full = m % 256 == 0 and n % 256 == 0 and k % 128 == 0 and k >= 256 and blocks > CUS
                    for pol in (([0, 1, 2, 6] if full else [0, 1, 2]) if (bm, bn) in PINGPONG and sk == 1 else lw):
                        rr = r if rasters is None else heuristic_raster(m, n, bm, bn, sk, stages=st)
                        out.append({"m1": bm, "n1": bn, "raster": rr, "stages": st, "splitk": sk, "policy": pol})
                        if (bm, bn) == (256, 256) and sk == 1 and blocks > 256 and 0 < blocks % 256 <= 64:
                            out.append({"m1": bm, "n1": bn, "raster": rr, "stages": st, "splitk": sk, "policy": pol, "tail": 1})
    if m <= 64 and k % 16 == 0 and k > 0:
        out.append({"m1": 16 if m <= 16 else (32 if m <= 32 else 64), "n1": 128, "raster": 1, "stages": 1, "splitk": 1, "policy": 0, "wsk": 1})
        if m <= 32:
            out.append({"m1": 16 if m <= 16 else 32, "n1": 128, "raster": 1, "stages": 3, "splitk": 1, "policy": 0, "wsk": 2})
    return out


BX_TILES = [(128, 256), (128, 128), (64, 256), (64, 128), (32, 128)]


def bx_raster(m, n, bm, bn, cus=256):
    tiles_m = -(-m // bm)
    tiles = tiles_m * -(-n // bn)
    wpc = 2 if bm * bn <= 64 * 128 else 1
    conc = min(max(1, tiles // 8), (cus // 8) * wpc)
    gm = 1
    while (gm * 2) * (gm * 2) * bm <= conc * bn and gm * 2 <= tiles_m:
        gm *= 2
    return gm


def candidates_bx(m, n, k, cus=256):
    kb = -(-k // 128)
    out = []
    for bm, bn in BX_TILES:
        if bm > 32 and bm >= 4 * max(m, 16):
            continue
        tiles = -(-m // bm) * -(-n // bn)
        rr = bx_raster(m, n, bm, bn, cus)
        splits = [1] + [sk for sk in (2, 3, 4, 6, 8, 16) if kb // sk >= 4 and tiles * sk <= 4 * cus and tiles < cus and sk * m * n * 4 <= (512 << 20)]
        for sk in splits:
            out.append({"m1": bm, "n1": bn, "raster": rr, "stages": 3, "splitk": sk, "policy": 7})
        if (bm, bn) == (128, 256):
            if tiles > cus:
                out.append({"m1": bm, "n1": bn, "raster": rr, "stages": 3, "splitk": 1, "policy": 7, "build": 8})
                if 0 < tiles % cus <= cus // 2:
                    out.append({"m1": bm, "n1": bn, "raster": rr, "stages": 3, "splitk": 1, "policy": 7, "tail": 1})
            if tiles % cus and kb >= 4:
                out.append({"m1": bm, "n1": bn, "raster": rr, "stages": 3, "splitk": 1, "policy": 7, "streamk": 1})
    if m <= 32 and k % 16 == 0 and kb >= 8:
        out.append({"m1": 16 if m <= 16 else 32, "n1": 128, "raster": 1, "stages": 3, "splitk": 1, "policy": 7, "wsk": 2})
    dt = -(-m // 64) * -(-n // 128)
    if 16 < m <= 512 and k % 16 == 0 and kb >= 4 and dt <= cus:
        smax = max(1, min(8, cus // dt, kb // 4))
        for sk in sorted({smax, max(1, (3 * smax) // 4), max(1, smax // 2)}):
            out.append({"m1": 64, "n1": 128, "raster": 1, "stages": 3, "splitk": sk, "policy": 7, "wsk": 2, "build": 10})
    return out


def bx_serial(p):
    return 6 if p.get("wsk") else (7 if p.get("streamk") else (5 if p.get("tail") else (4 if p["splitk"] > 1 else 0)))


MENU = [(256, 256, 4, 2, 2, (0, 1, 2, 6)), (128, 256, 2, 2, 2, (0, 2)), (256, 128, 4, 1, 2, (0, 2)), (128, 128, 2, 2, 2, (0, 2)),
        (64, 256, 1, 4, 2, (0, 2)), (64, 128, 1, 4, 2, (0,)), (128, 256, 2, 4, 2, (0, 2)), (128, 256, 2, 4, 3, (0,)),
        (128, 256, 2, 2, 3, (0, 4, 5)), (128, 128, 2, 2, 3, (0, 4, 5)), (64, 256, 1, 4, 3, (0, 4, 5)), (32, 256, 1, 4, 2, (0,)),
        (32, 128, 1, 4, 2, (0,)), (16, 256, 1, 4, 2, (0,)), (16, 128, 1, 4, 2, (0,)),
        (64, 128, 1, 4, 3, (0, 4, 5)), (32, 256, 1, 4, 3, (0,)), (32, 128, 1, 4, 3, (0,)), (16, 256, 1, 4, 3, (0,)), (16, 128, 1, 4, 3, (0, 4, 5))]
LDS_BYTES, ACC_REGS, CUS = 160 * 1024, 128, 256


def stage_bytes(bm, bn, waves):
    dnt = waves * 64
    a_rows = bm if bm * 8 >= dnt else dnt // 8
    return a_rows * 128 + bn * 128 + (-(-(bm + 8) // dnt) * dnt) * 4


def check_candidate(prob, c):
    bm, bn, wm, wn, st, pol, sk = c["m1"], c["n1"], c["wavesM"], c["wavesN"], c["stages"], c["policy"], c["splitk"]
    build = [v for v in MENU if v[:5] == (bm, bn, wm, wn, st)]
    if not build:
        return False, "no such build in the menu"
    if pol not in build[0][5]:
        return False, f"dispatch policy {pol} not compiled for this build"
    if stage_bytes(bm, bn, wm * wn) * st > LDS_BYTES:
        return False, "LDS"
    if bm * bn // (wm * wn * 64) > ACC_REGS:
        return False, "accumulator registers"
    kb = -(-prob["k"] // 128)
    if pol == 5:
        groups = prob["groups"] if prob["layout"] == "masked" else 1
        if sk != 1 or (prob["layout"] != "masked" and groups * -(-prob["m"] // bm) * -(-prob["n"] // bn) <= CUS):
            return False, "persistent form: more tiles than CUs, no split-K"
    if pol == 6 and (prob["layout"] != "dense" or prob["m"] % 256 or prob["n"] % 256 or prob["k"] % 128 or prob["k"] < 256 or
                     sk != 1 or (prob["m"] // 256) * (prob["n"] // 256) <= CUS):
        return False, "persistent continuous pipeline: dense rasters of full 256x256 tiles, more tiles than CUs"
    if prob["layout"] == "masked":
        need = 16 if prob["m"] <= 16 else 32 if prob["m"] <= 32 else 64 if prob["m"] <= 64 else 128
        if prob["m"] <= 128 and bm != need:
            return False, "masked layout: one tile row per expert (B is read once)"
        if sk != 1:
            return False, "split-K is dense only"
    elif prob["layout"] == "contiguous":
        tall = bm == 256 and bn == 256 and prob["rows_per_group"] >= 512
        if not tall and (bm > 128 or 128 % bm):
            return False, "contiguous layout: a tile must not straddle two group segments"
        if sk != 1:
            return False, "split-K is dense only"
    else:
        blocks = -(-prob["m"] // bm) * -(-prob["n"] // bn)
        if bm >= 2 * max(prob["m"], 16) and bm > 16:
            return False, "tile twice the problem"
        if sk > 1 and not (blocks * sk <= 1024 and kb // sk >= 4 and blocks < 192 and pol == 0):
            return False, "split-K needs few tiles, >= 4 k blocks per split and the plain loop"
    return True, ""


def grouped_candidates(prob):
    out = []
    for (bm, bn, wm, wn, st, pols) in MENU:
        for pol in pols:
            if pol == 1:
                continue
            c = {"m1": bm, "n1": bn, "wavesM": wm, "wavesN": wn, "stages": st, "policy": pol, "splitk": 1, "raster": 0}
            if check_candidate(prob, c)[0]:
                out.append(c)
    return out


def gen_data(m, n, k, seed=0):
    g = torch.Generator(device="cuda").manual_seed(seed)
    kp, np_ = -(-k // 128) * 128, -(-n // 128) * 128
    xa = torch.zeros((m, kp), device="cuda"); xa[:, :k] = torch.randn((m, k), device="cuda", generator=g)
    xb = torch.zeros((np_, kp), device="cuda"); xb[:n, :k] = torch.randn((n, k), device="cuda", generator=g)
    sa = xa.view(m, kp // 128, 128).abs().amax(2).clamp_min(1e-30) / 448
    qa = (xa.view(m, kp // 128, 128) / sa[..., None]).reshape(m, kp).to(torch.float8_e4m3fn)
    sb = xb.view(np_ // 128, 128, kp // 128, 128).abs().amax((1, 3)).clamp_min(1e-30) / 448
    qb = (xb.view(np_ // 128, 128, kp // 128, 128) / sb[:, None, :, None]).reshape(np_, kp).to(torch.float8_e4m3fn)
    da = (qa.float().view(m, kp // 128, 128) * sa[..., None]).reshape(m, kp)[:, :k]
    dbm = (qb.float().view(np_ // 128, 128, kp // 128, 128) * sb[:, None, :, None]).reshape(np_, kp)[:n, :k]
    golden = da @ dbm.T
    s_abs = da.abs() @ dbm.abs().T
    a = qa.view(torch.uint8)[:, :k].contiguous(); b = qb.view(torch.uint8)[:n, :k].contiguous()
    return a, sa.contiguous(), b, sb.contiguous(), golden, s_abs


def is_correct(golden, out, s_abs=None, policy="fast", short_k=False):
    from . import tolerance
    if s_abs is None:
        raise ValueError("is_correct needs S (gen_data's sixth return value): the bar is S-based")
    ok, rep = tolerance.check(out.float(), tolerance.bf16_round(golden), s_abs, policy=policy, short_k=short_k, golden_order="any")
    return ok, rep["frac_gt_2ulp"]


_TIMING_STREAM = []


def graph_us(fn, iters, replays=3, prewarm_ms=0.0):
    if not _TIMING_STREAM:
        _TIMING_STREAM.append(torch.cuda.Stream())
    side = _TIMING_STREAM[0]
    side.wait_stream(torch.cuda.current_stream())
    try:
        with torch.cuda.stream(side):
            fn()
        side.synchronize()
        g = torch.cuda.CUDAGraph()
        with torch.cuda.graph(g, stream=side):
            for _ in range(iters):
                fn()
    except Exception:
        torch.cuda.synchronize()
        return None
    import time as _time
    g.replay()
    torch.cuda.synchronize()
    t0 = _time.perf_counter()
    while (_time.perf_counter() - t0) * 1e3 < prewarm_ms:
        g.replay()
        torch.cuda.synchronize()
    e0 = torch.cuda.Event(enable_timing=True); e1 = torch.cuda.Event(enable_timing=True)
    e0.record()
    for _ in range(replays):
        g.replay()
    e1.record(); torch.cuda.synchronize()
    us = e0.elapsed_time(e1) * 1e3 / (iters * replays)
    del g
    return us


def time_us(fn, warm=3, iters=10, device_time=False):
    for _ in range(warm):
        fn()
    torch.cuda.synchronize()
    if device_time:
        us = graph_us(fn, iters)
        if us is not None:
            return us
    e0 = torch.cuda.Event(enable_timing=True); e1 = torch.cuda.Event(enable_timing=True)
    e0.record()
    for _ in range(iters):
        fn()
    e1.record(); torch.cuda.synchronize()
    return e0.elapsed_time(e1) * 1e3 / iters


COLD_MAX_M = 256
INFINITY_CACHE = 256 << 20


def benchmark_shape(shape, out_dir: Path, rank=0, num_processes=1, iters=10, rasters=None, prewarm_s=0.15, only_policy=None,
                    cold=False, versus_tuned=False, arith="fast"):
    import deepgemm_ascend_amd as dga
    m, n, k = shape
    bx = arith == "bf16_exact"
    cands = candidates_bx(m, n, k) if bx else candidates(m, n, k, rasters)
    if versus_tuned and not bx:
        t0 = dga.tiling(m, n, k)
        pick = {"m1": int(t0.m1), "n1": int(t0.n1), "raster": int(t0.swizzleOffset), "stages": 1 if t0.build == 1 else int(t0.stages),
                "splitk": int(t0.splitkFactor), "policy": int(t0.dispatchPolicyTag)}
        if t0.kernelSerial == 6:
            pick["wsk"] = 2 if (t0.build != 1 and m <= 32) else 1
        elif t0.kernelSerial == 5:
            pick["tail"] = 1
        cands = [pick] + [c for c in cands if c.get("wsk") and c != pick]
    if only_policy is not None:
        cands = [c for c in cands if c["policy"] == only_policy]
        if not cands:
            return None
    per = -(-len(cands) // num_processes)
    lo, hi = rank * per, min(len(cands), (rank + 1) * per)
    tagx = "bx_" if bx else ""
    res_path = out_dir / f"shape_{tagx}{m}_{n}_{k}_rank_{rank}.jsonl"
    ck_path = out_dir / f"shape_{tagx}{m}_{n}_{k}_rank_{rank}_checkpoint.jsonl"
    last = -1
    if ck_path.exists():
        try:
            last = json.loads(ck_path.read_text().strip().splitlines()[-1])["last_process_idx"]
        except Exception:
            last = -1
    a, sfa, b, sfb, golden, s_abs = gen_data(m, n, k)
    out = torch.empty((m, n), dtype=torch.bfloat16, device="cuda")
    import time as _time
    t_warm = dga.tiling(m, n, k, policy="bf16_exact" if bx else None)
    t0 = _time.perf_counter()
    while _time.perf_counter() - t0 < prewarm_s:
        for _ in range(20):
            dga.gemm_fp8_fp8_bf16_nt((a, sfa), (b, sfb), out, tiling_=t_warm, policy="bf16_exact" if bx else "fast")
        torch.cuda.synchronize()
    opbytes = m * k + n * k + 2 * m * n
    sets = [(a, sfa, b, sfb, out)]
    if cold and m <= COLD_MAX_M and opbytes < INFINITY_CACHE:
        for _ in range(min(16, max(3, -(-(320 << 20) // opbytes))) - 1):
            sets.append((a.clone(), sfa.clone(), b.clone(), sfb.clone(), torch.empty_like(out)))
    turn = [0]
    best = None
    for idx in range(lo, hi):
        if idx < last:
            continue
        p = cands[idx]
        if idx == last:
            with open(res_path, "a") as f:
                f.write(json.dumps(asdict(Result(idx, m, n, k, -1, -1, True, p))) + "\n")
            continue
        ck_path.write_text(json.dumps({"last_process_idx": idx}) + "\n")
        t = dga.tiling(m, n, k, policy="bf16_exact" if bx else None)
        t.m1, t.n1, t.swizzleOffset = p["m1"], p["n1"], p["raster"]
        t.stages, t.wavesM, t.wavesN, t.dispatchPolicyTag = (3 if p["stages"] == 1 else p["stages"]), 0, 0, p["policy"]
        t.build = p.get("build", 0) if bx else (1 if p.get("wsk") == 1 else 0)
        t.splitkFactor = p["splitk"]
        t.kernelSerial = bx_serial(p) if bx else (6 if p.get("wsk") else (5 if p.get("tail") else (4 if p["splitk"] > 1 else 0)))
        if dga.tiling_check(t) != 0:
            with open(res_path, "a") as f:
                f.write(json.dumps(asdict(Result(idx, m, n, k, -1, -1, True, dict(p, refused=1)))) + "\n")
            continue
        def fn():
            c = sets[turn[0] % len(sets)]
            turn[0] += 1
            dga.gemm_fp8_fp8_bf16_nt((c[0], c[1]), (c[2], c[3]), c[4], tiling_=t, policy="bf16_exact" if bx else None)
        turn[0] = 0
        fn(); torch.cuda.synchronize()
        ok, diff = is_correct(golden, out, s_abs, policy="bf16_exact" if bx else "fast", short_k=k < 128)
        n_it = -(-max(iters, 2 * len(sets)) // len(sets)) * len(sets)
        turn[0] = 0
        if ok and bx:
            for _ in range(max(3, len(sets))):
                fn()
            torch.cuda.synchronize()
            us = graph_us(fn, n_it, replays=5, prewarm_ms=25.0) or time_us(fn, warm=3, iters=n_it)
        else:
            us = time_us(fn, warm=max(3, len(sets)), iters=n_it, device_time=True) if ok else 999999999
        if len(sets) > 1:
            p = dict(p, cold_sets=len(sets))
        with open(res_path, "a") as f:
            f.write(json.dumps(asdict(Result(idx, m, n, k, us, diff, not ok, p))) + "\n")
        if ok and (best is None or us < best[0]):
            best = (us, p)
    ck_path.write_text(json.dumps({"last_process_idx": hi}) + "\n")
    return best


GROUPED_SHAPES = (
    [("masked", g, mm, n, k) for (n, k) in ((2048, 7168), (7168, 2048), (4096, 7168)) for g in (32, 256) for mm in (16, 64, 128)] +
    [("contiguous", g, r, n, k) for (n, k) in ((4096, 7168), (7168, 2048)) for (g, r) in ((32, 128), (8, 1024), (4, 4096))])


def benchmark_grouped(shape, out_dir: Path, iters=10, prewarm_s=0.15):
    import time as _time
    import deepgemm_ascend_amd as dga
    layout, groups, rows, n, k = shape
    gen = torch.Generator(device="cuda").manual_seed(0)
    rf = lambda sh: (lambda x: torch.where((x & 0x7F) == 0x7F, x & 0x80, x))(torch.randint(0, 256, sh, dtype=torch.uint8, device="cuda", generator=gen))
    kb, nb = k // 128, n // 128
    b = rf((groups, n, k)); sfb = torch.rand((groups, nb, kb), device="cuda", generator=gen) + 0.5
    if layout == "masked":
        prob = {"m": rows, "n": n, "k": k, "groups": groups, "layout": layout, "rows_per_group": rows}
        a = rf((groups, rows, k)); sfa = torch.rand((groups, rows, kb), device="cuda", generator=gen) + 0.5
        out = torch.empty((groups, rows, n), dtype=torch.bfloat16, device="cuda")
        masked = torch.full((groups,), rows, dtype=torch.int32, device="cuda")
        base = lambda: dga.tiling(rows, n, k, groups=groups, expected_m=rows)
        run = lambda t, strict=False: dga.m_grouped_gemm_fp8_fp8_bf16_nt_masked((a, sfa), (b, sfb), out, masked, rows, tiling_=t, strict=strict)
    else:
        msum = groups * rows
        prob = {"m": msum, "n": n, "k": k, "groups": groups, "layout": layout, "rows_per_group": rows}
        a = rf((msum, k)); sfa = torch.rand((msum, kb), device="cuda", generator=gen) + 0.5
        out = torch.empty((msum, n), dtype=torch.bfloat16, device="cuda")
        idx = torch.arange(groups, device="cuda", dtype=torch.int32).repeat_interleave(rows).contiguous()
        base = lambda: dga.tiling(msum, n, k, groups=groups, contiguous=True)
        run = lambda t, strict=False: dga.m_grouped_gemm_fp8_fp8_bf16_nt_contiguous((a, sfa), (b, sfb), out, idx, tiling_=t, strict=strict)
    from . import tolerance
    run(base(), strict=True); torch.cuda.synchronize()
    golden = out.float().clone()
    a_keep, b_keep = a.clone(), b.clone()
    a &= 0x7F; b &= 0x7F
    run(base(), strict=True); torch.cuda.synchronize()
    s_abs = out.float().clone()
    a.copy_(a_keep); b.copy_(b_keep)
    del a_keep, b_keep
    t0 = _time.perf_counter()
    while _time.perf_counter() - t0 < prewarm_s:
        run(base()); torch.cuda.synchronize()
    tag = f"{layout}_{groups}x{rows}_{n}_{k}"
    res_path = out_dir / f"shape_{tag}_rank_0.jsonl"
    best = None
    for i, c in enumerate(grouped_candidates(prob)):
        t = base()
        t.m1, t.n1, t.wavesM, t.wavesN, t.stages, t.dispatchPolicyTag = c["m1"], c["n1"], c["wavesM"], c["wavesN"], c["stages"], c["policy"]
        t.splitkFactor, t.kernelSerial = 1, 0
        tiles = -(-prob["m"] // c["m1"]) * -(-n // c["n1"])
        t.blockDim = tiles * (groups if layout == "masked" else (2 if c["m1"] == 256 else 1))
        c = dict(c, raster=int(t.swizzleOffset), groups=groups, layout=layout, rows_per_group=rows)
        try:
            run(t); torch.cuda.synchronize()
            ok, rep = tolerance.check(out.float(), golden, s_abs, policy="fast", short_k=True)
            ratio = rep["frac_gt_2ulp"]
            us = time_us(lambda: run(t), iters=iters) if ok else 999999999
        except Exception:
            ok, ratio, us = False, -1.0, 999999999
        with open(res_path, "a") as f:
            f.write(json.dumps(asdict(Result(i, prob["m"], n, k, us, ratio, not ok, c))) + "\n")
        if ok and (best is None or us < best[0]):
            best = (us, c)
    return prob, best


FAST_CSV_HEAD = ("m,n,k,m1,n1,k1,kernelSerial,paddingTagA,paddingTagB,paddingTagC,blockDim,"
                 "splitkFactor,stages,swizzleOffset,wavesM,wavesN,dispatchPolicyTag\n")
GROUPED_CSV_HEAD = FAST_CSV_HEAD.strip() + ",groups,contiguous\n"
FULL_CSV_HEAD = GROUPED_CSV_HEAD.strip() + ",build\n"


def fast_row(m, n, k, p):
    serial = 6 if p.get("wsk") else (5 if p.get("tail") else (4 if p["splitk"] > 1 else 0))
    blocks = -(-m // p["m1"]) * -(-n // p["n1"]) * p["splitk"]
    if p.get("tail"):
        blocks = blocks - blocks % 256 + 4 * (blocks % 256)
    return f"{m},{n},{k},{p['m1']},{p['n1']},128,{serial},0,0,0,{blocks},{p['splitk']},{p['stages']},{p['raster']},0,0,{p['policy']}\n"


def grouped_row(prob, c):
    tiles = -(-prob["m"] // c["m1"]) * -(-prob["n"] // c["n1"])
    contiguous = 1 if prob["layout"] == "contiguous" else 0
    block_dim = tiles * (1 if contiguous else prob["groups"]) * (2 if contiguous and c["m1"] == 256 else 1)
    return (f"{prob['m']},{prob['n']},{prob['k']},{c['m1']},{c['n1']},128,0,0,0,0,{block_dim},1,{c['stages']},"
            f"{c['raster']},{c['wavesM']},{c['wavesN']},{c['policy']},{prob['groups']},{contiguous}\n")


def bx_row(m, n, k, p, cus=256):
    tiles = -(-m // p["m1"]) * -(-n // p["n1"])
    serial = bx_serial(p)
    block_dim = tiles * p["splitk"]
    if serial == 5:
        block_dim = tiles - tiles % cus + 4 * (tiles % cus)
    elif serial == 7:
        block_dim = cus
    elif serial == 6 and p.get("build") != 10:
        block_dim = min(-(-n // 16), cus)
    return (f"{m},{n},{k},{p['m1']},{p['n1']},128,{serial},0,0,0,{block_dim},{p['splitk']},3,{p['raster']},0,0,7,1,0,{p.get('build', 0)}\n")


def write_bx_rows(path, winners):
    path = Path(path)
    lines = path.read_text().splitlines(keepends=True) if path.exists() else []
    if not lines:
        lines = [FULL_CSV_HEAD]
    head = lines[0].strip().split(",")
    if "build" not in head:
        assert head == GROUPED_CSV_HEAD.strip().split(","), "the cache file must carry the CDNA4 and group columns"
        lines = [FULL_CSV_HEAD] + [ln.rstrip("\n") + ",0\n" for ln in lines[1:] if ln.strip()]
    keys = {(m, n, k) for (m, n, k), _ in winners}
    def is_old_bx(ln):
        c = ln.strip().split(",")
        return len(c) >= 19 and (int(c[0]), int(c[1]), int(c[2])) in keys and (int(c[16]) & 15) == 7 and int(c[17]) <= 1 and int(c[18]) == 0
    lines = [lines[0]] + [ln for ln in lines[1:] if ln.strip() and not is_old_bx(ln)]
    lines += [bx_row(m, n, k, p) for (m, n, k), p in winners]
    path.write_text("".join(lines))


def main(argv=None):
    ap = argparse.ArgumentParser()
    ap.add_argument("--out", default="sweep_out")
    ap.add_argument("--rank", type=int, default=int(os.environ.get("RANK", 0)))
    ap.add_argument("--num-processes", type=int, default=int(os.environ.get("WORLD_SIZE", 1)))
    ap.add_argument("--shapes", nargs="*", default=None, help="M,N,K ...")
    ap.add_argument("--iters", type=int, default=10)
    ap.add_argument("--cache-csv", default=None, help="append winners to this tiling-cache CSV")
    ap.add_argument("--grid", type=int, default=0, help="sweep this many random shapes (predictor training set)")
    ap.add_argument("--grid-seed", type=int, default=0)
    ap.add_argument("--prewarm-ms", type=float, default=150.0, help="clock pre-warm in front of every shape's candidates")
    ap.add_argument("--heuristic-raster", action="store_true",
                    help="one raster per candidate (the heuristic's) instead of the raster sweep")
    ap.add_argument("--only-policy", type=int, default=None, help="time only the candidates of this dispatchPolicyTag")
    ap.add_argument("--versus-tuned", action="store_true",
                    help="time only the operator's current pick and the workgroup split-K builds (a supplementary sweep)")
    ap.add_argument("--cold", action="store_true",
                    help=f"shapes with M <= {COLD_MAX_M}: rotate operand sets past the Infinity Cache (decode weights are never warm)")
    ap.add_argument("--arith", default="fast", choices=["fast", "bf16_exact"],
                    help="the arithmetic policy whose menu is swept: the fast path's (dispatchPolicyTag 0-6) or the in-contract "
                         "bf16-exact policy's (7: the operator's default; winners become tag-7 rows of the cache CSV)")
    ap.add_argument("--grouped", action="store_true",
                    help="sweep the masked / contiguous grouped shapes (GROUPED_SHAPES) instead of the dense list")
    ap.add_argument("--grouped-shapes", nargs="*", default=None,
                    help="with --grouped: layout,groups,rows,n,k ... instead of GROUPED_SHAPES (layout: masked | contiguous)")
    a = ap.parse_args(argv)
    torch.cuda.set_device(a.rank % max(1, torch.cuda.device_count()))
    out_dir = Path(a.out); out_dir.mkdir(parents=True, exist_ok=True)
    if a.grouped:
        rows_out = []
        gshapes = GROUPED_SHAPES
        if a.grouped_shapes:
            gshapes = [(s.split(",")[0],) + tuple(int(x) for x in s.split(",")[1:]) for s in a.grouped_shapes]
        for shape in gshapes[a.rank::a.num_processes]:
            prob, best = benchmark_grouped(shape, out_dir, a.iters, a.prewarm_ms / 1e3)
            if best:
                us, c = best
                print(json.dumps({"shape": list(shape), "best_us": round(us, 2), **c}), flush=True)
                rows_out.append(grouped_row(prob, c))
        if a.cache_csv and rows_out:
            new = not Path(a.cache_csv).exists()
            with open(a.cache_csv, "a") as f:
                if new:
                    f.write(GROUPED_CSV_HEAD)
                f.writelines(rows_out)
        return
    shapes = [[int(x) for x in s.split(",")] for s in a.shapes] if a.shapes else SHAPE_GROUP
    if a.grid:
        shapes = grid_shapes(a.grid, a.grid_seed)
    winners = []
    for shape in shapes:
        best = benchmark_shape(shape, out_dir, a.rank, a.num_processes, a.iters, [0] if a.heuristic_raster else None,
                               a.prewarm_ms / 1e3, a.only_policy, a.cold, a.versus_tuned, a.arith)
        if best:
            us, p = best
            m, n, k = shape
            print(json.dumps({"shape": shape, "best_us": round(us, 2), "tflops": round(2.0 * m * n * k / us / 1e6, 1), **p}), flush=True)
            winners.append((shape, p))
    if a.cache_csv and winners and a.arith == "bf16_exact":
        write_bx_rows(a.cache_csv, winners)
    elif a.cache_csv and winners:
        new = not Path(a.cache_csv).exists()
        with open(a.cache_csv, "a") as f:
            if new:
                f.write(FAST_CSV_HEAD)
            f.writelines(fast_row(m, n, k, p) for (m, n, k), p in winners)


if __name__ == "__main__":
    main()
```

Measured before the change: 1193.

## Route dense bf16x 128x256 GEMMs through a staggered persistent kernel specialization

Moves the grouped kernel body into a shared include and instantiates a DENSE specialization that drops group and masked-M lookups. It also pins the fill offsets in scalar registers and reuses precomputed own-wave offsets. The dispatcher now sends dense bf16-output 128x256 tiles to this staggered persistent schedule by default when the tile count reaches the CU count and K has at least 4 blocks. This happens before the existing persistent path, with the aim of overlapping wave halves' MFMA and refill work. The risk is that the default route changes for large dense shapes and may not beat the tuned persistent kernel.

```diff
diff --git a/deepgemm_ascend_amd/csrc/dga_launch.hip b/deepgemm_ascend_amd/csrc/dga_launch.hip
--- a/deepgemm_ascend_amd/csrc/dga_launch.hip
+++ b/deepgemm_ascend_amd/csrc/dga_launch.hip
@@ -191,6 +191,7 @@
     int wsk = env_int("DGA_WSK", -1), wsk_dma = env_int("DGA_WSK_DMA", -1);
     int pingpong = env_int("DGA_PINGPONG", -1);
     int bx_persist = env_int("DGA_BF16X_PERSIST", -1), bx_grouped = env_int("DGA_BX_GROUPED", -1);
+    int bx_dense_stagger = env_int("DGA_BX_DENSE_STAGGER", -1);
 };
 static const Switches &env()
 {
@@ -471,6 +472,11 @@
         if (rc != DGA_E_TILING) return rc;
     }
     const bool pays = tiles > cus;
+    if (vx->bm == 128 && vx->bn == 256 && dense && c.kind == Out::Bf16 && t.kernelSerial == DGA_KERNEL_COMMON && t.build == DGA_BUILD_DEFAULT &&
+        (env().bx_dense_stagger >= 0 ? env().bx_dense_stagger != 0 : (env().bx_persist < 0 && tiles >= cus && p.kb_n >= 4))) {
+        rc = launch_bf16x_grouped(p, c.stream);
+        if (rc != DGA_E_TILING) return rc;
+    }
     if (vx->bm == 128 && vx->bn == 256 &&
         (env().bx_persist >= 0 ? env().bx_persist != 0 : (t.build == DGA_BUILD_BX_PERSISTENT || (t.build != DGA_BUILD_BX_ONE_TILE && pays)))) {
         rc = launch_bf16x_persistent(p, c.kind, c.stream);
diff --git a/deepgemm_ascend_amd/csrc/dga_launch_menu_l.hip b/deepgemm_ascend_amd/csrc/dga_launch_menu_l.hip
--- a/deepgemm_ascend_amd/csrc/dga_launch_menu_l.hip
+++ b/deepgemm_ascend_amd/csrc/dga_launch_menu_l.hip
@@ -13,16 +13,29 @@
     return launch_kernel<gemm_fp8_bf16x_grouped_kernel<KTAIL, BNT, STAG, IDX>>(grid, Cfg::NT, kLds, stream, p);
 }
 
+template <bool KTAIL, bool STAG>
+static int launch_bf16x_dense_stagger_one(const GemmParams &p, hipStream_t stream)
+{
+    typedef GemmCfg<128, 256, 2, 4, 3> Cfg;
+    const int64_t tiles = static_cast<int64_t>(p.tiles_m) * p.tiles_n;
+    const unsigned grid = static_cast<unsigned>(std::min<int64_t>(tiles, device_cus()));
+    return launch_kernel<gemm_fp8_bf16x_grouped_kernel_dense<KTAIL, STAG>>(grid, Cfg::NT, Cfg::LDS_BYTES, stream, p);
+}
+
 int launch_bf16x_grouped(const GemmParams &p, hipStream_t stream)
 {
     if (p.tail_sub || p.m_indices || p.launch_tiles > 0 || p.splitk > 1 || p.kb_n < 2) return DGA_E_TILING;
     const bool nt = p.b_nt != 0;
 #ifdef DGA_BXG_KNOBS
     if (const char *e = std::getenv("DGA_BXG_KNOB"); e && (std::atoi(e) & 2)) {
+        if (p.groups == 1 && !p.masked_m && !p.row_index)
+            return p.k % 128 ? launch_bf16x_dense_stagger_one<true, false>(p, stream) : launch_bf16x_dense_stagger_one<false, false>(p, stream);
         if (p.k % 128) return nt ? launch_bf16x_grouped_one<true, true, false>(p, stream) : launch_bf16x_grouped_one<true, false, false>(p, stream);
         return nt ? launch_bf16x_grouped_one<false, true, false>(p, stream) : launch_bf16x_grouped_one<false, false, false>(p, stream);
     }
 #endif
+    if (p.groups == 1 && !p.masked_m && !p.row_index)
+        return p.k % 128 ? launch_bf16x_dense_stagger_one<true, true>(p, stream) : launch_bf16x_dense_stagger_one<false, true>(p, stream);
     if (p.row_index) {
         if (p.k % 128) return nt ? launch_bf16x_grouped_one<true, true, true, true>(p, stream) : launch_bf16x_grouped_one<true, false, true, true>(p, stream);
         return nt ? launch_bf16x_grouped_one<false, true, true, true>(p, stream) : launch_bf16x_grouped_one<false, false, true, true>(p, stream);
diff --git a/deepgemm_ascend_amd/csrc/gemm_fp8_bf16x_grouped_body.inc b/deepgemm_ascend_amd/csrc/gemm_fp8_bf16x_grouped_body.inc
--- /dev/null
+++ b/deepgemm_ascend_amd/csrc/gemm_fp8_bf16x_grouped_body.inc
@@ -0,0 +1,407 @@
+    typedef GemmCfg<128, 256, 2, 4, 3> Cfg;
+    constexpr int BM = Cfg::kBM, BN = Cfg::kBN, WN = Cfg::kWN, TM = Cfg::TM, TN = Cfg::TN, DNT = Cfg::DNT;
+    constexpr int NL = Cfg::LOADS_PER_STAGE, LAGT = 2, RING = 4, NT = Cfg::NT;
+    static_assert(Cfg::NT == 512 && DNT == 512 && TM == 4 && TN == 4 && Cfg::SC_ITERS == 1 && Cfg::STAGES == 3, "the grouped schedule");
+    typedef __bf16 v8bf __attribute__((ext_vector_type(8)));
+    extern __shared__ __attribute__((aligned(16))) uint8_t smem[];
+
+    const int tid = threadIdx.x, lane = tid & 63;
+    const int wave = __builtin_amdgcn_readfirstlane(tid >> 6);
+    const int wm = wave / WN, wn = wave % WN;
+    const int li = lane & 15, kg = lane >> 4;
+    const int KB = p.kb_n;
+
+    const int tiles_per_group = p.tiles_m * p.tiles_n;
+    const int total = p.groups * tiles_per_group;
+    int first = 0, count = total, step = gridDim.x, slot = blockIdx.x;
+    if (p.xcd_remap) {
+        const int xcd = blockIdx.x & 7, q = total >> 3, r = total & 7;
+        first = xcd < r ? xcd * (q + 1) : r * (q + 1) + (xcd - r) * q;
+        count = q + (xcd < r ? 1 : 0);
+        step = ((int)gridDim.x - xcd + 7) >> 3;
+        slot = blockIdx.x >> 3;
+    }
+    struct Tile { int g, M, m0, n0; };
+    typedef const __attribute__((address_space(4))) int32_t *const_i32_ptr;
+    const const_i32_ptr masked_m_c = (const_i32_ptr)p.masked_m;
+    auto seek = [&](int &local, Tile &t) -> bool {
+        for (; local < count; local += step) {
+            const int tile = first + local;
+            const int g = DENSE ? 0 : tile / tiles_per_group;
+            const int t_in = tile - g * tiles_per_group;
+            const int gm = p.raster_group;
+            const int per = gm * p.tiles_n;
+            const int band = t_in / per;
+            const int row0 = band * gm;
+            const int rows = min(p.tiles_m - row0, gm);
+            const int loc = t_in - band * per;
+            const int tm = row0 + loc % rows, tn = loc / rows;
+            const int M = DENSE ? p.m : (p.masked_m ? min(masked_m_c[g], p.m) : p.m);
+            const int m0 = tm * BM;
+            if (m0 >= M) continue;
+            t.g = g; t.M = M; t.m0 = m0; t.n0 = tn * BN;
+            return true;
+        }
+        return false;
+    };
+
+    const uint32_t lds0 = (uint32_t)(uintptr_t)(lptr_t)smem;
+    constexpr uint32_t kOutOfRange = 0x80000000u;
+    const int a_col = ((tid & 7) ^ swz_a(tid >> 3)) * 16;
+    const int b_col = ((tid & 7) ^ swz_b(tid >> 3)) * 16;
+    v4i a_rsrc, b_rsrc;
+    uint32_t a_voff[Cfg::A_ITERS], b_voff[Cfg::B_ITERS];
+    const float *sc_src;
+    int kbf = 0;
+    bool fill_valid = true;
+    constexpr bool indexed = INDEXED;
+    static_assert(Cfg::A_ITERS == 2, "partner slot: two A offsets and the scale pointer");
+    uint32_t *const pslot = reinterpret_cast<uint32_t *>(smem + Cfg::LDS_BYTES) + (tid & (DNT / 2 - 1)) * 4;
+    auto a_off_of = [&](const Tile &t, int it, int td) -> uint32_t {
+        const int row = (it * DNT + td) >> 3;
+        if (row >= t.M - t.m0) return kOutOfRange;
+        const uint32_t r = indexed ? (uint32_t)p.row_index[(int64_t)t.g * p.m + t.m0 + row] : (uint32_t)row;
+        return r * (uint32_t)p.lda + a_col;
+    };
+    auto b_off_of = [&](const Tile &t, int it, int td) -> uint32_t {
+        const int row = (it * DNT + td) >> 3;
+        return (uint32_t)min(row, p.n - 1 - t.n0) * (uint32_t)p.ldb + b_col;
+    };
+    auto sc_of = [&](const Tile &t, int td) -> const float * {
+        const float *SFA = p.sfa + (int64_t)t.g * p.sfa_gs, *SFB = p.sfb + (int64_t)t.g * p.sfb_gs;
+        if (td >= BM) return SFB + (int64_t)min(t.n0 / 128 + min(td - BM, 7), p.nb_n - 1) * p.kb_n;
+        const int mr = min(t.m0 + td, t.M - 1);
+        return SFA + (indexed ? p.row_index[(int64_t)t.g * p.m + mr] : (int64_t)mr) * p.sfa_ld;
+    };
+    Tile T{}, F{};
+    auto set_fill = [&](const Tile &t) {
+        a_rsrc = indexed ? make_rsrc(p.a, p.a_bytes)
+                         : make_rsrc(p.a + (int64_t)t.g * p.a_gs + (int64_t)t.m0 * p.lda, (int64_t)(t.M - t.m0) * p.lda);
+        b_rsrc = make_rsrc(p.b + (int64_t)t.g * p.b_gs + (int64_t)t.n0 * p.ldb, (int64_t)(p.n - t.n0) * p.ldb);
+#pragma unroll
+        for (int it = 0; it < Cfg::A_ITERS; ++it) a_voff[it] = a_off_of(t, it, tid);
+#pragma unroll
+        for (int it = 0; it < Cfg::B_ITERS; ++it) b_voff[it] = b_off_of(t, it, tid);
+        sc_src = sc_of(t, tid);
+        if constexpr (INDEXED) {
+            if (wm == 1) {
+                const uint64_t ps = (uint64_t)(uintptr_t)sc_of(t, tid - DNT / 2);
+                *reinterpret_cast<v4i *>(pslot) = v4i{(int)a_off_of(t, 0, tid - DNT / 2), (int)a_off_of(t, 1, tid - DNT / 2), (int)(uint32_t)ps, (int)(uint32_t)(ps >> 32)};
+            }
+        }
+    };
+    auto refill = [&](int idx, int stage, auto sc) {
+        constexpr int S = decltype(sc)::value;
+        const int w = wave - 4 * S, td = tid - S * (DNT / 2);
+        auto opaque = [](uint32_t v) __attribute__((always_inline)) -> uint32_t {
+            if constexpr (DENSE) asm volatile("" : "+s"(v));
+            return v;
+        };
+        const uint32_t sa = opaque(lds0 + stage * Cfg::STAGE_BYTES + w * 1024);
+        const int k0 = kbf * 128;
+        if (idx < Cfg::A_ITERS) {
+            uint32_t voff = (DENSE && !S) ? a_voff[idx] : fill_valid ? (S ? (INDEXED ? pslot[idx] : a_off_of(F, idx, td)) : a_voff[idx]) : kOutOfRange;
+            if constexpr (KTAIL) voff = (k0 + a_col < p.k) ? voff : kOutOfRange;
+            dma16(voff, a_rsrc, (uint32_t)k0, sa + idx * DNT * 16);
+        } else if (idx < Cfg::A_ITERS + Cfg::B_ITERS) {
+            const int it = idx - Cfg::A_ITERS;
+            uint32_t voff = (DENSE && !S) ? b_voff[it] : fill_valid ? (S ? b_off_of(F, it, td) : b_voff[it]) : kOutOfRange;
+            if constexpr (KTAIL) voff = (k0 + b_col < p.k) ? voff : kOutOfRange;
+            if constexpr (BNT) dma16_nt(voff, b_rsrc, (uint32_t)k0, sa + Cfg::A_BYTES + it * DNT * 16);
+            else dma16(voff, b_rsrc, (uint32_t)k0, sa + Cfg::A_BYTES + it * DNT * 16);
+        } else {
+            const float *src = S ? (INDEXED ? reinterpret_cast<const float *>((uintptr_t)*reinterpret_cast<const uint64_t *>(pslot + 2)) : sc_of(F, td)) : sc_src;
+            if constexpr (DENSE) dma4(src + (!S || fill_valid ? kbf : KB - 1), opaque(lds0 + stage * Cfg::STAGE_BYTES + w * 256) + Cfg::A_BYTES + Cfg::B_BYTES);
+            else dma4(src + (fill_valid ? kbf : KB - 1), lds0 + stage * Cfg::STAGE_BYTES + Cfg::A_BYTES + Cfg::B_BYTES + w * 256);
+        }
+    };
+    constexpr std::integral_constant<int, 0> kOwn{};
+    constexpr std::integral_constant<int, 1> kPartner{};
+
+    const int a_row = wm * (BM / Cfg::kWM) + li;
+    const int a_off0 = a_row * 128 + ((kg ^ swz_a(a_row)) * 16);
+    const int a_off1 = a_row * 128 + (((kg + 4) ^ swz_a(a_row)) * 16);
+    const int b_row = wn * (BN / WN) + 8 * (li >> 2) + (li & 3);
+    const int b_off0 = Cfg::A_BYTES + b_row * 128 + ((kg ^ swz_b(b_row)) * 16);
+    const int b_off1 = Cfg::A_BYTES + b_row * 128 + (((kg + 4) ^ swz_b(b_row)) * 16);
+    const int sa_off = Cfg::A_BYTES + Cfg::B_BYTES + (wm * (BM / Cfg::kWM) + li) * 4;
+    const int sb_off = Cfg::A_BYTES + Cfg::B_BYTES + (BM + (wn * (BN / WN)) / 128) * 4;
+
+    v4f acc[TM][TN];
+    v4f part[RING];
+    v4i afx[TM][4], bfx[2][4];
+    v4i braw[2], araw[2][2];
+    float s_cur[TM], s_old[TM];
+
+    auto wait_all_but = [&](auto base, int extra) {
+        constexpr int B = decltype(base)::value;
+        if (extra >= 8) wait_vmcnt<B + 8>();
+        else if (extra >= 6) wait_vmcnt<B + 6>();
+        else if (extra >= 4) wait_vmcnt<B + 4>();
+        else if (extra >= 2) wait_vmcnt<B + 2>();
+        else wait_vmcnt<B>();
+    };
+    auto wait_landed = [&](int younger, int extra) {
+        if (younger >= 2 * NL) wait_all_but(std::integral_constant<int, 2 * NL>{}, extra);
+        else if (younger >= NL) wait_all_but(std::integral_constant<int, NL>{}, extra);
+        else wait_all_but(std::integral_constant<int, 0>{}, extra);
+    };
+
+    int local = slot;
+    if (!seek(local, T)) return;
+    F = T;
+    set_fill(F);
+#pragma unroll
+    for (int d = 0; d < 2; ++d) {
+#pragma unroll
+        for (int idx = 0; idx < NL; ++idx) refill(idx, d, kOwn);
+        ++kbf;
+    }
+    int cur = 0;
+    DGA_STAMP_DECL
+    DGA_STAMP_CLOCK(6, 7);
+    DGA_STAMP_START();
+    int stores_pending = 0;
+    int younger = NL;
+
+    auto advance_fill = [&]() {
+        if (kbf == KB) {
+            local += step;
+            fill_valid = seek(local, F);
+            if (fill_valid) set_fill(F);
+            else if constexpr (DENSE) {
+#pragma unroll
+                for (int it = 0; it < Cfg::A_ITERS; ++it) a_voff[it] = kOutOfRange;
+#pragma unroll
+                for (int it = 0; it < Cfg::B_ITERS; ++it) b_voff[it] = kOutOfRange;
+            }
+            kbf = 0;
+        }
+    };
+
+    auto run_tile = [&](auto Lc, auto lonec, auto stagc) __attribute__((always_inline)) {
+        constexpr int L = decltype(Lc)::value;
+        constexpr bool lone = decltype(lonec)::value;
+        constexpr bool STAG = decltype(stagc)::value;
+        constexpr int G = 4 * (L > 0 ? L : 1);
+        constexpr int TILES = (L > 0 ? L : 1) * TN;
+        constexpr int SP = L > 0 ? L : 1;
+        constexpr int HALF = 2 * TILES;
+        static_assert(1 + (NL - 1) * SP < HALF, "the refill fits half a block");
+        static_assert(!(STAG && (lone || L == 0)), "a staggered wave multiplies and issues its own pieces");
+        if constexpr (L > 0) {
+#pragma unroll
+            for (int i = 0; i < L; ++i)
+#pragma unroll
+                for (int j = 0; j < TN; ++j) acc[i][j] = v4f{0.f, 0.f, 0.f, 0.f};
+#pragma unroll
+            for (int i = 0; i < RING; ++i) part[i] = v4f{0.f, 0.f, 0.f, 0.f};
+#pragma unroll
+            for (int i = 0; i < L; ++i) s_old[i] = 0.f;
+        }
+        auto head = [&](const uint8_t *sc) __attribute__((always_inline)) {
+            araw[0][0] = *(const v4i *)(sc + a_off0);
+            araw[0][1] = *(const v4i *)(sc + a_off1);
+            braw[0] = *(const v4i *)(sc + b_off0);
+            braw[1] = *(const v4i *)(sc + b_off1);
+            if constexpr (L > 1) {
+                araw[1][0] = *(const v4i *)(sc + a_off0 + 2048);
+                araw[1][1] = *(const v4i *)(sc + a_off1 + 2048);
+            }
+            const float sfb0 = *(const float *)(sc + sb_off);
+            float sa[L > 0 ? L : 1];
+#pragma unroll
+            for (int i = 0; i < L; ++i) sa[i] = *(const float *)(sc + sa_off + i * 64);
+            __builtin_amdgcn_sched_barrier(0);
+#pragma unroll
+            for (int c = 0; c < 8; ++c) bx_convert(braw, bfx[0], c);
+            braw[0] = *(const v4i *)(sc + b_off0 + b_frag_off(1));
+#pragma unroll
+            for (int c = 8; c < 16; ++c) bx_convert(braw, bfx[0], c);
+            braw[1] = *(const v4i *)(sc + b_off1 + b_frag_off(1));
+#pragma unroll
+            for (int c = 0; c < 16; ++c) bx_convert(araw[0], afx[0], c);
+            if constexpr (L > 2) {
+                araw[0][0] = *(const v4i *)(sc + a_off0 + 2 * 2048);
+                araw[0][1] = *(const v4i *)(sc + a_off1 + 2 * 2048);
+            }
+#pragma unroll
+            for (int i = 0; i < L; ++i) s_cur[i] = sa[i] * sfb0;
+            __builtin_amdgcn_sched_barrier(0);
+        };
+        auto gaps = [&](auto u0c, auto u1c, auto refillc, const uint8_t *sc, int fill) __attribute__((always_inline)) {
+            constexpr int U0 = decltype(u0c)::value, U1 = decltype(u1c)::value;
+            constexpr bool REFILL = decltype(refillc)::value;
+#pragma unroll
+            for (int u = U0; u < U1; ++u) {
+                const int t = u >> 2, q = u & 3, nt = t / L, mt = t % L, g = u % G;
+                part[t % RING] = __builtin_amdgcn_mfma_f32_16x16x32_bf16(
+                    __builtin_bit_cast(v8bf, bfx[nt & 1][q]), __builtin_bit_cast(v8bf, afx[mt][q]),
+                    q == 0 ? v4f{0.f, 0.f, 0.f, 0.f} : part[t % RING], 0, 0, 0);
+                __builtin_amdgcn_sched_barrier(0);
+                if (REFILL && u - U0 >= 1 && (u - U0 - 1) % SP == 0 && (u - U0 - 1) / SP < NL) refill((u - U0 - 1) / SP, fill, kOwn);
+                if (nt == 0 && mt + 1 < L) {
+#pragma unroll
+                    for (int c = 0; c < 4; ++c) bx_convert(araw[(mt + 1) & 1], afx[mt + 1], 4 * q + c);
+                    if (q == 3 && mt + 3 < L) {
+                        araw[(mt + 1) & 1][0] = *(const v4i *)(sc + a_off0 + (mt + 3) * 2048);
+                        araw[(mt + 1) & 1][1] = *(const v4i *)(sc + a_off1 + (mt + 3) * 2048);
+                    }
+                }
+                if (nt + 1 < TN) {
+#pragma unroll
+                    for (int c = 16 * g / G; c < 16 * (g + 1) / G; ++c) bx_convert(braw, bfx[(nt + 1) & 1], c);
+                    if (nt + 2 < TN) {
+                        if (g == G / 2 - 1) braw[0] = *(const v4i *)(sc + b_off0 + b_frag_off(nt + 2));
+                        if (g == G - 1) braw[1] = *(const v4i *)(sc + b_off1 + b_frag_off(nt + 2));
+                    }
+                }
+                {
+                    const int j = t >= LAGT ? t - LAGT : TILES + t - LAGT, jn = j / L, jm = j % L;
+                    const float sv = t >= LAGT ? s_cur[jm] : s_old[jm];
+                    acc[jm][jn][q] = __builtin_fmaf(part[j % RING][q], sv, acc[jm][jn][q]);
+                }
+                __builtin_amdgcn_sched_barrier(0);
+            }
+        };
+        constexpr std::integral_constant<int, 0> kU0{};
+        constexpr std::integral_constant<int, HALF> kUh{};
+        constexpr std::integral_constant<int, 4 * TILES> kU1{};
+        auto end_of_block = [&]() {
+#pragma unroll
+            for (int i = 0; i < L; ++i) s_old[i] = s_cur[i];
+        };
+        auto top = [&](int kb) __attribute__((always_inline)) -> int {
+            DGA_STAMP(0);
+            if (DENSE && younger == NL && (kb >= 2 || stores_pending == 0)) wait_vmcnt<NL>();
+            else wait_landed(younger, kb < 2 ? stores_pending : 0);
+            DGA_STAMP(1);
+            __builtin_amdgcn_s_barrier();
+            asm volatile("" ::: "memory");
+            DGA_STAMP(2);
+            advance_fill();
+            return cur >= 1 ? cur - 1 : 2;
+        };
+        auto next_block = [&]() {
+            ++kbf;
+            cur = cur == 2 ? 0 : cur + 1;
+        };
+        if constexpr (STAG) {
+            {
+                const int fill = top(0);
+                younger = NL;
+#pragma unroll
+                for (int idx = 0; idx < NL; ++idx) refill(idx, fill, kOwn);
+                const uint8_t *sc = smem + cur * Cfg::STAGE_BYTES;
+                head(sc);
+                gaps(kU0, kUh, std::false_type{}, sc, fill);
+                next_block();
+            }
+            for (int kb = 1; kb < KB; ++kb) {
+                const int fill = top(kb);
+                const uint8_t *sc = smem + cur * Cfg::STAGE_BYTES;
+                gaps(kUh, kU1, std::true_type{}, sc, fill);
+                end_of_block();
+                head(sc);
+                DGA_STAMP(3);
+                gaps(kU0, kUh, std::false_type{}, sc, fill);
+                DGA_STAMP(4);
+                next_block();
+            }
+            gaps(kUh, kU1, std::false_type{}, smem, 0);
+            end_of_block();
+        } else {
+            for (int kb = 0; kb < KB; ++kb) {
+                const int fill = top(kb);
+                if constexpr (L == 0) {
+#pragma unroll
+                    for (int idx = 0; idx < NL; ++idx) {
+                        if (lone) refill(idx, fill, kPartner);
+                        refill(idx, fill, kOwn);
+                    }
+                    younger = lone ? 2 * NL : NL;
+                } else {
+                    younger = lone ? 0 : NL;
+                    const uint8_t *sc = smem + cur * Cfg::STAGE_BYTES;
+                    head(sc);
+                    DGA_STAMP(3);
+                    if constexpr (lone) gaps(kU0, kU1, std::false_type{}, sc, fill);
+                    else gaps(kU0, kU1, std::true_type{}, sc, fill);
+                    end_of_block();
+                    DGA_STAMP(4);
+                }
+                next_block();
+            }
+        }
+        stores_pending = 0;
+        if constexpr (L > 0) {
+#pragma unroll
+            for (int t = 0; t < LAGT; ++t) {
+                const int j = TILES + t - LAGT, jn = j / L, jm = j % L;
+#pragma unroll
+                for (int q = 0; q < 4; ++q) acc[jm][jn][q] = __builtin_fmaf(part[j % RING][q], s_old[jm], acc[jm][jn][q]);
+            }
+            uint16_t *C = p.out + (int64_t)T.g * p.c_gs;
+            const int m_row = T.m0 + wm * (BM / Cfg::kWM) + li;
+            const int n_base = T.n0 + wn * (BN / WN) + 8 * kg;
+            const bool vec_ok = ((p.ldc & 7) == 0) && ((((uintptr_t)C) & 15) == 0);
+            if (vec_ok && T.n0 + BN <= p.n) stores_pending = 2 * L;
+#pragma unroll
+            for (int mt = 0; mt < L; ++mt) {
+                const int m = m_row + mt * 16;
+                if (m >= T.M) continue;
+                uint16_t *crow = C + (indexed ? p.row_index[(int64_t)T.g * p.m + m] : (int64_t)m) * p.ldc;
+#pragma unroll
+                for (int j = 0; j < TN / 2; ++j) {
+                    const int n = n_base + 32 * j;
+                    const v4f lo = acc[mt][2 * j], hi = acc[mt][2 * j + 1];
+                    const v2bf h0 = __builtin_convertvector(v2f{lo.x, lo.y}, v2bf);
+                    const v2bf h1 = __builtin_convertvector(v2f{lo.z, lo.w}, v2bf);
+                    const v2bf h2 = __builtin_convertvector(v2f{hi.x, hi.y}, v2bf);
+                    const v2bf h3 = __builtin_convertvector(v2f{hi.z, hi.w}, v2bf);
+                    const v4i pk = v4i{__builtin_bit_cast(int, h0), __builtin_bit_cast(int, h1),
+                                       __builtin_bit_cast(int, h2), __builtin_bit_cast(int, h3)};
+                    if (vec_ok && n + 8 <= p.n) {
+                        if (p.out_nt == 1) asm volatile("global_store_dwordx4 %0, %1, off nt" :: "v"(crow + n), "v"(pk) : "memory");
+                        else if (p.out_nt == 2) asm volatile("global_store_dwordx4 %0, %1, off sc0 sc1" :: "v"(crow + n), "v"(pk) : "memory");
+                        else if (p.out_nt == 3) asm volatile("global_store_dwordx4 %0, %1, off sc0 sc1 nt" :: "v"(crow + n), "v"(pk) : "memory");
+                        else asm volatile("global_store_dwordx4 %0, %1, off" :: "v"(crow + n), "v"(pk) : "memory");
+                    } else {
+                        const uint16_t *e = (const uint16_t *)&pk;
+#pragma unroll
+                        for (int q = 0; q < 8; ++q)
+                            if (n + q < p.n) crow[n + q] = e[q];
+                    }
+                }
+            }
+        }
+    };
+
+    for (;;) {
+        const int rows = T.M - T.m0 - wm * (BM / Cfg::kWM);
+        const int L = rows <= 0 ? 0 : (rows >= 64 ? 4 : (rows + 15) >> 4);
+        const bool lone = T.M - T.m0 <= BM / Cfg::kWM;
+        constexpr std::true_type yes{};
+        constexpr std::false_type no{};
+        if (lone) {
+            if (L == 0) run_tile(std::integral_constant<int, 0>{}, yes, no);
+            else if (L == 1) run_tile(std::integral_constant<int, 1>{}, yes, no);
+            else if (L == 2) run_tile(std::integral_constant<int, 2>{}, yes, no);
+            else if (L == 3) run_tile(std::integral_constant<int, 3>{}, yes, no);
+            else run_tile(std::integral_constant<int, 4>{}, yes, no);
+        } else if (wm == 0) {
+            run_tile(std::integral_constant<int, 4>{}, no, no);
+        } else {
+            constexpr std::integral_constant<bool, STAGGER> st{};
+            if (L == 1) run_tile(std::integral_constant<int, 1>{}, no, st);
+            else if (L == 2) run_tile(std::integral_constant<int, 2>{}, no, st);
+            else if (L == 3) run_tile(std::integral_constant<int, 3>{}, no, st);
+            else run_tile(std::integral_constant<int, 4>{}, no, st);
+        }
+        if (!fill_valid) break;
+        T = F;
+    }
+    DGA_STAMP(5);
+    DGA_STAMP_CLOCK(6, 7);
+    DGA_STAMP_FLUSH();
+    wait_vmcnt<0>();
diff --git a/deepgemm_ascend_amd/csrc/gemm_fp8_bf16x_grouped_kernel.hpp b/deepgemm_ascend_amd/csrc/gemm_fp8_bf16x_grouped_kernel.hpp
--- a/deepgemm_ascend_amd/csrc/gemm_fp8_bf16x_grouped_kernel.hpp
+++ b/deepgemm_ascend_amd/csrc/gemm_fp8_bf16x_grouped_kernel.hpp
@@ -7,401 +7,16 @@
 __global__ void __launch_bounds__(512) __attribute__((amdgpu_waves_per_eu(2, 2)))
 gemm_fp8_bf16x_grouped_kernel(const GemmParams p)
 {
-    typedef GemmCfg<128, 256, 2, 4, 3> Cfg;
-    constexpr int BM = Cfg::kBM, BN = Cfg::kBN, WN = Cfg::kWN, TM = Cfg::TM, TN = Cfg::TN, DNT = Cfg::DNT;
-    constexpr int NL = Cfg::LOADS_PER_STAGE, LAGT = 2, RING = 4, NT = Cfg::NT;
-    static_assert(Cfg::NT == 512 && DNT == 512 && TM == 4 && TN == 4 && Cfg::SC_ITERS == 1 && Cfg::STAGES == 3, "the grouped schedule");
-    typedef __bf16 v8bf __attribute__((ext_vector_type(8)));
-    extern __shared__ __attribute__((aligned(16))) uint8_t smem[];
+    constexpr bool DENSE = false;
+#include "gemm_fp8_bf16x_grouped_body.inc"
+}
 
-    const int tid = threadIdx.x, lane = tid & 63;
-    const int wave = __builtin_amdgcn_readfirstlane(tid >> 6);
-    const int wm = wave / WN, wn = wave % WN;
-    const int li = lane & 15, kg = lane >> 4;
-    const int KB = p.kb_n;
-
-    const int tiles_per_group = p.tiles_m * p.tiles_n;
-    const int total = p.groups * tiles_per_group;
-    int first = 0, count = total, step = gridDim.x, slot = blockIdx.x;
-    if (p.xcd_remap) {
-        const int xcd = blockIdx.x & 7, q = total >> 3, r = total & 7;
-        first = xcd < r ? xcd * (q + 1) : r * (q + 1) + (xcd - r) * q;
-        count = q + (xcd < r ? 1 : 0);
-        step = ((int)gridDim.x - xcd + 7) >> 3;
-        slot = blockIdx.x >> 3;
-    }
-    struct Tile { int g, M, m0, n0; };
-    typedef const __attribute__((address_space(4))) int32_t *const_i32_ptr;
-    const const_i32_ptr masked_m_c = (const_i32_ptr)p.masked_m;
-    auto seek = [&](int &local, Tile &t) -> bool {
-        for (; local < count; local += step) {
-            const int tile = first + local;
-            const int g = tile / tiles_per_group;
-            const int t_in = tile - g * tiles_per_group;
-            const int gm = p.raster_group;
-            const int per = gm * p.tiles_n;
-            const int band = t_in / per;
-            const int row0 = band * gm;
-            const int rows = min(p.tiles_m - row0, gm);
-            const int loc = t_in - band * per;
-            const int tm = row0 + loc % rows, tn = loc / rows;
-            const int M = p.masked_m ? min(masked_m_c[g], p.m) : p.m;
-            const int m0 = tm * BM;
-            if (m0 >= M) continue;
-            t.g = g; t.M = M; t.m0 = m0; t.n0 = tn * BN;
-            return true;
-        }
-        return false;
-    };
-
-    const uint32_t lds0 = (uint32_t)(uintptr_t)(lptr_t)smem;
-    constexpr uint32_t kOutOfRange = 0x80000000u;
-    const int a_col = ((tid & 7) ^ swz_a(tid >> 3)) * 16;
-    const int b_col = ((tid & 7) ^ swz_b(tid >> 3)) * 16;
-    v4i a_rsrc, b_rsrc;
-    uint32_t a_voff[Cfg::A_ITERS], b_voff[Cfg::B_ITERS];
-    const float *sc_src;
-    int kbf = 0;
-    bool fill_valid = true;
-    constexpr bool indexed = INDEXED;
-    static_assert(Cfg::A_ITERS == 2, "partner slot: two A offsets and the scale pointer");
-    uint32_t *const pslot = reinterpret_cast<uint32_t *>(smem + Cfg::LDS_BYTES) + (tid & (DNT / 2 - 1)) * 4;
-    auto a_off_of = [&](const Tile &t, int it, int td) -> uint32_t {
-        const int row = (it * DNT + td) >> 3;
-        if (row >= t.M - t.m0) return kOutOfRange;
-        const uint32_t r = indexed ? (uint32_t)p.row_index[(int64_t)t.g * p.m + t.m0 + row] : (uint32_t)row;
-        return r * (uint32_t)p.lda + a_col;
-    };
-    auto b_off_of = [&](const Tile &t, int it, int td) -> uint32_t {
-        const int row = (it * DNT + td) >> 3;
-        return (uint32_t)min(row, p.n - 1 - t.n0) * (uint32_t)p.ldb + b_col;
-    };
-    auto sc_of = [&](const Tile &t, int td) -> const float * {
-        const float *SFA = p.sfa + (int64_t)t.g * p.sfa_gs, *SFB = p.sfb + (int64_t)t.g * p.sfb_gs;
-        if (td >= BM) return SFB + (int64_t)min(t.n0 / 128 + min(td - BM, 7), p.nb_n - 1) * p.kb_n;
-        const int mr = min(t.m0 + td, t.M - 1);
-        return SFA + (indexed ? p.row_index[(int64_t)t.g * p.m + mr] : (int64_t)mr) * p.sfa_ld;
-    };
-    Tile T{}, F{};
-    auto set_fill = [&](const Tile &t) {
-        a_rsrc = indexed ? make_rsrc(p.a, p.a_bytes)
-                         : make_rsrc(p.a + (int64_t)t.g * p.a_gs + (int64_t)t.m0 * p.lda, (int64_t)(t.M - t.m0) * p.lda);
-        b_rsrc = make_rsrc(p.b + (int64_t)t.g * p.b_gs + (int64_t)t.n0 * p.ldb, (int64_t)(p.n - t.n0) * p.ldb);
-#pragma unroll
-        for (int it = 0; it < Cfg::A_ITERS; ++it) a_voff[it] = a_off_of(t, it, tid);
-#pragma unroll
-        for (int it = 0; it < Cfg::B_ITERS; ++it) b_voff[it] = b_off_of(t, it, tid);
-        sc_src = sc_of(t, tid);
-        if constexpr (INDEXED) {
-            if (wm == 1) {
-                const uint64_t ps = (uint64_t)(uintptr_t)sc_of(t, tid - DNT / 2);
-                *reinterpret_cast<v4i *>(pslot) = v4i{(int)a_off_of(t, 0, tid - DNT / 2), (int)a_off_of(t, 1, tid - DNT / 2), (int)(uint32_t)ps, (int)(uint32_t)(ps >> 32)};
-            }
-        }
-    };
-    auto refill = [&](int idx, int stage, auto sc) {
-        constexpr int S = decltype(sc)::value;
-        const int w = wave - 4 * S, td = tid - S * (DNT / 2);
-        const uint32_t sa = lds0 + stage * Cfg::STAGE_BYTES + w * 1024;
-        const int k0 = kbf * 128;
-        if (idx < Cfg::A_ITERS) {
-            uint32_t voff = fill_valid ? (S ? (INDEXED ? pslot[idx] : a_off_of(F, idx, td)) : a_voff[idx]) : kOutOfRange;
-            if constexpr (KTAIL) voff = (k0 + a_col < p.k) ? voff : kOutOfRange;
-            dma16(voff, a_rsrc, (uint32_t)k0, sa + idx * DNT * 16);
-        } else if (idx < Cfg::A_ITERS + Cfg::B_ITERS) {
-            const int it = idx - Cfg::A_ITERS;
-            uint32_t voff = fill_valid ? (S ? b_off_of(F, it, td) : b_voff[it]) : kOutOfRange;
-            if constexpr (KTAIL) voff = (k0 + b_col < p.k) ? voff : kOutOfRange;
-            if constexpr (BNT) dma16_nt(voff, b_rsrc, (uint32_t)k0, sa + Cfg::A_BYTES + it * DNT * 16);
-            else dma16(voff, b_rsrc, (uint32_t)k0, sa + Cfg::A_BYTES + it * DNT * 16);
-        } else {
-            const float *src = S ? (INDEXED ? reinterpret_cast<const float *>((uintptr_t)*reinterpret_cast<const uint64_t *>(pslot + 2)) : sc_of(F, td)) : sc_src;
-            dma4(src + (fill_valid ? kbf : KB - 1), lds0 + stage * Cfg::STAGE_BYTES + Cfg::A_BYTES + Cfg::B_BYTES + w * 256);
-        }
-    };
-    constexpr std::integral_constant<int, 0> kOwn{};
-    constexpr std::integral_constant<int, 1> kPartner{};
-
-    const int a_row = wm * (BM / Cfg::kWM) + li;
-    const int a_off0 = a_row * 128 + ((kg ^ swz_a(a_row)) * 16);
-    const int a_off1 = a_row * 128 + (((kg + 4) ^ swz_a(a_row)) * 16);
-    const int b_row = wn * (BN / WN) + 8 * (li >> 2) + (li & 3);
-    const int b_off0 = Cfg::A_BYTES + b_row * 128 + ((kg ^ swz_b(b_row)) * 16);
-    const int b_off1 = Cfg::A_BYTES + b_row * 128 + (((kg + 4) ^ swz_b(b_row)) * 16);
-    const int sa_off = Cfg::A_BYTES + Cfg::B_BYTES + (wm * (BM / Cfg::kWM) + li) * 4;
-    const int sb_off = Cfg::A_BYTES + Cfg::B_BYTES + (BM + (wn * (BN / WN)) / 128) * 4;
-
-    v4f acc[TM][TN];
-    v4f part[RING];
-    v4i afx[TM][4], bfx[2][4];
-    v4i braw[2], araw[2][2];
-    float s_cur[TM], s_old[TM];
-
-    auto wait_all_but = [&](auto base, int extra) {
-        constexpr int B = decltype(base)::value;
-        if (extra >= 8) wait_vmcnt<B + 8>();
-        else if (extra >= 6) wait_vmcnt<B + 6>();
-        else if (extra >= 4) wait_vmcnt<B + 4>();
-        else if (extra >= 2) wait_vmcnt<B + 2>();
-        else wait_vmcnt<B>();
-    };
-    auto wait_landed = [&](int younger, int extra) {
-        if (younger >= 2 * NL) wait_all_but(std::integral_constant<int, 2 * NL>{}, extra);
-        else if (younger >= NL) wait_all_but(std::integral_constant<int, NL>{}, extra);
-        else wait_all_but(std::integral_constant<int, 0>{}, extra);
-    };
-
-    int local = slot;
-    if (!seek(local, T)) return;
-    F = T;
-    set_fill(F);
-#pragma unroll
-    for (int d = 0; d < 2; ++d) {
-#pragma unroll
-        for (int idx = 0; idx < NL; ++idx) refill(idx, d, kOwn);
-        ++kbf;
-    }
-    int cur = 0;
-    DGA_STAMP_DECL
-    DGA_STAMP_CLOCK(6, 7);
-    DGA_STAMP_START();
-    int stores_pending = 0;
-    int younger = NL;
-
-    auto advance_fill = [&]() {
-        if (kbf == KB) {
-            local += step;
-            fill_valid = seek(local, F);
-            if (fill_valid) set_fill(F);
-            kbf = 0;
-        }
-    };
-
-    auto run_tile = [&](auto Lc, auto lonec, auto stagc) __attribute__((always_inline)) {
-        constexpr int L = decltype(Lc)::value;
-        constexpr bool lone = decltype(lonec)::value;
-        constexpr bool STAG = decltype(stagc)::value;
-        constexpr int G = 4 * (L > 0 ? L : 1);
-        constexpr int TILES = (L > 0 ? L : 1) * TN;
-        constexpr int SP = L > 0 ? L : 1;
-        constexpr int HALF = 2 * TILES;
-        static_assert(1 + (NL - 1) * SP < HALF, "the refill fits half a block");
-        static_assert(!(STAG && (lone || L == 0)), "a staggered wave multiplies and issues its own pieces");
-        if constexpr (L > 0) {
-#pragma unroll
-            for (int i = 0; i < L; ++i)
-#pragma unroll
-                for (int j = 0; j < TN; ++j) acc[i][j] = v4f{0.f, 0.f, 0.f, 0.f};
-#pragma unroll
-            for (int i = 0; i < RING; ++i) part[i] = v4f{0.f, 0.f, 0.f, 0.f};
-#pragma unroll
-            for (int i = 0; i < L; ++i) s_old[i] = 0.f;
-        }
-        auto head = [&](const uint8_t *sc) __attribute__((always_inline)) {
-            araw[0][0] = *(const v4i *)(sc + a_off0);
-            araw[0][1] = *(const v4i *)(sc + a_off1);
-            braw[0] = *(const v4i *)(sc + b_off0);
-            braw[1] = *(const v4i *)(sc + b_off1);
-            if constexpr (L > 1) {
-                araw[1][0] = *(const v4i *)(sc + a_off0 + 2048);
-                araw[1][1] = *(const v4i *)(sc + a_off1 + 2048);
-            }
-            const float sfb0 = *(const float *)(sc + sb_off);
-            float sa[L > 0 ? L : 1];
-#pragma unroll
-            for (int i = 0; i < L; ++i) sa[i] = *(const float *)(sc + sa_off + i * 64);
-            __builtin_amdgcn_sched_barrier(0);
-#pragma unroll
-            for (int c = 0; c < 8; ++c) bx_convert(braw, bfx[0], c);
-            braw[0] = *(const v4i *)(sc + b_off0 + b_frag_off(1));
-#pragma unroll
-            for (int c = 8; c < 16; ++c) bx_convert(braw, bfx[0], c);
-            braw[1] = *(const v4i *)(sc + b_off1 + b_frag_off(1));
-#pragma unroll
-            for (int c = 0; c < 16; ++c) bx_convert(araw[0], afx[0], c);
-            if constexpr (L > 2) {
-                araw[0][0] = *(const v4i *)(sc + a_off0 + 2 * 2048);
-                araw[0][1] = *(const v4i *)(sc + a_off1 + 2 * 2048);
-            }
-#pragma unroll
-            for (int i = 0; i < L; ++i) s_cur[i] = sa[i] * sfb0;
-            __builtin_amdgcn_sched_barrier(0);
-        };
-        auto gaps = [&](auto u0c, auto u1c, auto refillc, const uint8_t *sc, int fill) __attribute__((always_inline)) {
-            constexpr int U0 = decltype(u0c)::value, U1 = decltype(u1c)::value;
-            constexpr bool REFILL = decltype(refillc)::value;
-#pragma unroll
-            for (int u = U0; u < U1; ++u) {
-                const int t = u >> 2, q = u & 3, nt = t / L, mt = t % L, g = u % G;
-                part[t % RING] = __builtin_amdgcn_mfma_f32_16x16x32_bf16(
-                    __builtin_bit_cast(v8bf, bfx[nt & 1][q]), __builtin_bit_cast(v8bf, afx[mt][q]),
-                    q == 0 ? v4f{0.f, 0.f, 0.f, 0.f} : part[t % RING], 0, 0, 0);
-                __builtin_amdgcn_sched_barrier(0);
-                if (REFILL && u - U0 >= 1 && (u - U0 - 1) % SP == 0 && (u - U0 - 1) / SP < NL) refill((u - U0 - 1) / SP, fill, kOwn);
-                if (nt == 0 && mt + 1 < L) {
-#pragma unroll
-                    for (int c = 0; c < 4; ++c) bx_convert(araw[(mt + 1) & 1], afx[mt + 1], 4 * q + c);
-                    if (q == 3 && mt + 3 < L) {
-                        araw[(mt + 1) & 1][0] = *(const v4i *)(sc + a_off0 + (mt + 3) * 2048);
-                        araw[(mt + 1) & 1][1] = *(const v4i *)(sc + a_off1 + (mt + 3) * 2048);
-                    }
-                }
-                if (nt + 1 < TN) {
-#pragma unroll
-                    for (int c = 16 * g / G; c < 16 * (g + 1) / G; ++c) bx_convert(braw, bfx[(nt + 1) & 1], c);
-                    if (nt + 2 < TN) {
-                        if (g == G / 2 - 1) braw[0] = *(const v4i *)(sc + b_off0 + b_frag_off(nt + 2));
-                        if (g == G - 1) braw[1] = *(const v4i *)(sc + b_off1 + b_frag_off(nt + 2));
-                    }
-                }
-                {
-                    const int j = t >= LAGT ? t - LAGT : TILES + t - LAGT, jn = j / L, jm = j % L;
-                    const float sv = t >= LAGT ? s_cur[jm] : s_old[jm];
-                    acc[jm][jn][q] = __builtin_fmaf(part[j % RING][q], sv, acc[jm][jn][q]);
-                }
-                __builtin_amdgcn_sched_barrier(0);
-            }
-        };
-        constexpr std::integral_constant<int, 0> kU0{};
-        constexpr std::integral_constant<int, HALF> kUh{};
-        constexpr std::integral_constant<int, 4 * TILES> kU1{};
-        auto end_of_block = [&]() {
-#pragma unroll
-            for (int i = 0; i < L; ++i) s_old[i] = s_cur[i];
-        };
-        auto top = [&](int kb) __attribute__((always_inline)) -> int {
-            DGA_STAMP(0);
-            wait_landed(younger, kb < 2 ? stores_pending : 0);
-            DGA_STAMP(1);
-            __builtin_amdgcn_s_barrier();
-            asm volatile("" ::: "memory");
-            DGA_STAMP(2);
-            advance_fill();
-            return cur >= 1 ? cur - 1 : 2;
-        };
-        auto next_block = [&]() {
-            ++kbf;
-            cur = cur == 2 ? 0 : cur + 1;
-        };
-        if constexpr (STAG) {
-            {
-                const int fill = top(0);
-                younger = NL;
-#pragma unroll
-                for (int idx = 0; idx < NL; ++idx) refill(idx, fill, kOwn);
-                const uint8_t *sc = smem + cur * Cfg::STAGE_BYTES;
-                head(sc);
-                gaps(kU0, kUh, std::false_type{}, sc, fill);
-                next_block();
-            }
-            for (int kb = 1; kb < KB; ++kb) {
-                const int fill = top(kb);
-                const uint8_t *sc = smem + cur * Cfg::STAGE_BYTES;
-                gaps(kUh, kU1, std::true_type{}, sc, fill);
-                end_of_block();
-                head(sc);
-                DGA_STAMP(3);
-                gaps(kU0, kUh, std::false_type{}, sc, fill);
-                DGA_STAMP(4);
-                next_block();
-            }
-            gaps(kUh, kU1, std::false_type{}, smem, 0);
-            end_of_block();
-        } else {
-            for (int kb = 0; kb < KB; ++kb) {
-                const int fill = top(kb);
-                if constexpr (L == 0) {
-#pragma unroll
-                    for (int idx = 0; idx < NL; ++idx) {
-                        if (lone) refill(idx, fill, kPartner);
-                        refill(idx, fill, kOwn);
-                    }
-                    younger = lone ? 2 * NL : NL;
-                } else {
-                    younger = lone ? 0 : NL;
-                    const uint8_t *sc = smem + cur * Cfg::STAGE_BYTES;
-                    head(sc);
-                    DGA_STAMP(3);
-                    if constexpr (lone) gaps(kU0, kU1, std::false_type{}, sc, fill);
-                    else gaps(kU0, kU1, std::true_type{}, sc, fill);
-                    end_of_block();
-                    DGA_STAMP(4);
-                }
-                next_block();
-            }
-        }
-        stores_pending = 0;
-        if constexpr (L > 0) {
-#pragma unroll
-            for (int t = 0; t < LAGT; ++t) {
-                const int j = TILES + t - LAGT, jn = j / L, jm = j % L;
-#pragma unroll
-                for (int q = 0; q < 4; ++q) acc[jm][jn][q] = __builtin_fmaf(part[j % RING][q], s_old[jm], acc[jm][jn][q]);
-            }
-            uint16_t *C = p.out + (int64_t)T.g * p.c_gs;
-            const int m_row = T.m0 + wm * (BM / Cfg::kWM) + li;
-            const int n_base = T.n0 + wn * (BN / WN) + 8 * kg;
-            const bool vec_ok = ((p.ldc & 7) == 0) && ((((uintptr_t)C) & 15) == 0);
-            if (vec_ok && T.n0 + BN <= p.n) stores_pending = 2 * L;
-#pragma unroll
-            for (int mt = 0; mt < L; ++mt) {
-                const int m = m_row + mt * 16;
-                if (m >= T.M) continue;
-                uint16_t *crow = C + (indexed ? p.row_index[(int64_t)T.g * p.m + m] : (int64_t)m) * p.ldc;
-#pragma unroll
-                for (int j = 0; j < TN / 2; ++j) {
-                    const int n = n_base + 32 * j;
-                    const v4f lo = acc[mt][2 * j], hi = acc[mt][2 * j + 1];
-                    const v2bf h0 = __builtin_convertvector(v2f{lo.x, lo.y}, v2bf);
-                    const v2bf h1 = __builtin_convertvector(v2f{lo.z, lo.w}, v2bf);
-                    const v2bf h2 = __builtin_convertvector(v2f{hi.x, hi.y}, v2bf);
-                    const v2bf h3 = __builtin_convertvector(v2f{hi.z, hi.w}, v2bf);
-                    const v4i pk = v4i{__builtin_bit_cast(int, h0), __builtin_bit_cast(int, h1),
-                                       __builtin_bit_cast(int, h2), __builtin_bit_cast(int, h3)};
-                    if (vec_ok && n + 8 <= p.n) {
-                        if (p.out_nt == 1) asm volatile("global_store_dwordx4 %0, %1, off nt" :: "v"(crow + n), "v"(pk) : "memory");
-                        else if (p.out_nt == 2) asm volatile("global_store_dwordx4 %0, %1, off sc0 sc1" :: "v"(crow + n), "v"(pk) : "memory");
-                        else if (p.out_nt == 3) asm volatile("global_store_dwordx4 %0, %1, off sc0 sc1 nt" :: "v"(crow + n), "v"(pk) : "memory");
-                        else asm volatile("global_store_dwordx4 %0, %1, off" :: "v"(crow + n), "v"(pk) : "memory");
-                    } else {
-                        const uint16_t *e = (const uint16_t *)&pk;
-#pragma unroll
-                        for (int q = 0; q < 8; ++q)
-                            if (n + q < p.n) crow[n + q] = e[q];
-                    }
-                }
-            }
-        }
-    };
-
-    for (;;) {
-        const int rows = T.M - T.m0 - wm * (BM / Cfg::kWM);
-        const int L = rows <= 0 ? 0 : (rows >= 64 ? 4 : (rows + 15) >> 4);
-        const bool lone = T.M - T.m0 <= BM / Cfg::kWM;
-        constexpr std::true_type yes{};
-        constexpr std::false_type no{};
-        if (lone) {
-            if (L == 0) run_tile(std::integral_constant<int, 0>{}, yes, no);
-            else if (L == 1) run_tile(std::integral_constant<int, 1>{}, yes, no);
-            else if (L == 2) run_tile(std::integral_constant<int, 2>{}, yes, no);
-            else if (L == 3) run_tile(std::integral_constant<int, 3>{}, yes, no);
-            else run_tile(std::integral_constant<int, 4>{}, yes, no);
-        } else if (wm == 0) {
-            run_tile(std::integral_constant<int, 4>{}, no, no);
-        } else {
-            constexpr std::integral_constant<bool, STAGGER> st{};
-            if (L == 1) run_tile(std::integral_constant<int, 1>{}, no, st);
-            else if (L == 2) run_tile(std::integral_constant<int, 2>{}, no, st);
-            else if (L == 3) run_tile(std::integral_constant<int, 3>{}, no, st);
-            else run_tile(std::integral_constant<int, 4>{}, no, st);
-        }
-        if (!fill_valid) break;
-        T = F;
-    }
-    DGA_STAMP(5);
-    DGA_STAMP_CLOCK(6, 7);
-    DGA_STAMP_FLUSH();
-    wait_vmcnt<0>();
+template <bool KTAIL, bool STAGGER = true>
+__global__ void __launch_bounds__(512) __attribute__((amdgpu_waves_per_eu(2, 2)))
+gemm_fp8_bf16x_grouped_kernel_dense(const GemmParams p)
+{
+    constexpr bool DENSE = true, BNT = false, INDEXED = false;
+#include "gemm_fp8_bf16x_grouped_body.inc"
 }
 
 }
diff --git a/deepgemm_ascend_amd/harness/sweep.py b/deepgemm_ascend_amd/harness/sweep.py
--- a/deepgemm_ascend_amd/harness/sweep.py
+++ b/deepgemm_ascend_amd/harness/sweep.py
@@ -103,6 +103,9 @@
     return gm
 
 
+DENSE_STAGGER_CANDIDATE = False
+
+
 def candidates_bx(m, n, k, cus=256):
     kb = -(-k // 128)
     out = []
@@ -119,6 +122,8 @@
                 out.append({"m1": bm, "n1": bn, "raster": rr, "stages": 3, "splitk": 1, "policy": 7, "build": 8})
                 if 0 < tiles % cus <= cus // 2:
                     out.append({"m1": bm, "n1": bn, "raster": rr, "stages": 3, "splitk": 1, "policy": 7, "tail": 1})
+            if DENSE_STAGGER_CANDIDATE and tiles >= cus and kb >= 2:
+                out.append({"m1": bm, "n1": bn, "raster": rr, "stages": 3, "splitk": 1, "policy": 7, "build": 9})
             if tiles % cus and kb >= 4:
                 out.append({"m1": bm, "n1": bn, "raster": rr, "stages": 3, "splitk": 1, "policy": 7, "streamk": 1})
     if m <= 32 and k % 16 == 0 and kb >= 8:
```

Result: no change. 1213 (median of 3 runs) (+1.7%).
